# johndpope/MegaPortrait-hack

Hardware: AMD Instinct MI355X
Metric: Gbase fwd hot-slice frames/sec @512^2 (96ch 16x64x64 volume) (higher is better)
Workload: dtype f16x3 (fp32 in/out, operands split into 2 f16 halves, 3 f16 MFMAs per product, fp32 accumulate; 3x3x3 convs that fill the chip run in the F(2,3) Winograd domain along W)

## Files before the change

include/mphip.h:

```cpp
#ifndef MPHIP_H
#define MPHIP_H

#include <stddef.h>
#include <stdint.h>

#define MPHIP_RANGE_FLOATS 4100

#ifdef __cplusplus
extern "C" {
#endif

#define MPHIP_OK 0
#define MPHIP_EINVAL (-1)
#define MPHIP_ELAUNCH (-2)
#define MPHIP_EWORKSPACE (-3)

#define MPHIP_ABI_VERSION 25
int mphip_version(void);
int mphip_graph_memsets_to_kernels(void *graph, int *replaced);
int mphip_graph_memset_nodes_left(void *graph, int *left);

int mphip_build_flags(void);
const char *mphip_last_error(void);

int mphip_rt_theta(const float *rotation_deg, const float *translation, float *theta, int B, int invert,
                   void *stream);

int mphip_warp_field_compose(const float *theta, const float *em, const float *base_tbl, float *w,
                             float *rt_out, float *em_out, int B, int eD, int eH, int eW, int G,
                             void *stream);

size_t mphip_warp_workspace_bytes(int B, int D, int H, int W);
size_t mphip_warp_corner_image_bytes(int B, int C);
int mphip_warp_corner_image(const float *v, void *img, size_t img_bytes, int B, int C, int D, int H, int W, void *stream);
int mphip_warp_volume_coords_img(const float *v, const float *coords, float *out, float *out_range, int B, int C, int D, int H, int W,
                                 void *workspace, size_t workspace_bytes, const void *img, void *stream);
int mphip_warp_volume(const float *v, const float *field, const float *lin_d, const float *lin_h,
                      const float *lin_w, float *out, float *coords_out, int32_t *idx_out, float *out_range, int B,
                      int C, int D, int H, int W, int fD, int fH, int fW, void *workspace, size_t workspace_bytes,
                      void *stream);

int mphip_warp_volume_dsum(const float *v, const float *field, const float *lin_d, const float *lin_h,
                           const float *lin_w, float *out, int B, int C, int D, int H, int W, int fD,
                           int fH, int fW, void *workspace, size_t workspace_bytes, void *stream);
int mphip_warp_volume_dsum_shared(const float *v, const float *field, const float *lin_d, const float *lin_h,
                                  const float *lin_w, float *out, int B, int C, int D, int H, int W, int fD,
                                  int fH, int fW, void *workspace, size_t workspace_bytes, void *stream);

int mphip_conv3d_supported(int N, int Ci, int Co, int D, int H, int W, int k, int precision);
size_t mphip_packed_weight_bytes(int Co, int Ci, int k, int precision);
int mphip_pack_conv_weight(const float *w_oidhw, void *w_packed, int Co, int Ci, int k, int precision,
                           void *stream);
size_t mphip_conv3d_workspace_bytes(int N, int Ci, int Co, int D, int H, int W, int k, int precision);
int mphip_absmax_range(const float *x, size_t n, float *range, void *stream);
int mphip_conv3d_fwd(const float *x, const float *x_range, const void *w_packed, const float *bias, float *y, int N,
                     int Ci, int Co, int D, int H, int W, int k, int precision, void *workspace,
                     size_t workspace_bytes, void *stream);

size_t mphip_conv3d_gn_workspace_bytes(int N, int Ci, int Co, int D, int H, int W, int k, int precision,
                                       int gn_groups);
int mphip_conv3d_gn_fwd(const float *x, const float *x_range, const void *w_packed, const float *bias, float *y, float *gn_stats,
                        int N, int Ci, int Co, int D, int H, int W, int k, int precision, int gn_groups,
                        float gn_eps, void *workspace, size_t workspace_bytes, void *stream);

int mphip_groupnorm_affine_table(const float *stats, const float *gamma, const float *beta, const float *w2,
                                 const float *b2, float *table, float *out_range, int N, int C, int S, int G,
                                 void *stream);
int mphip_conv3d_gn_table_fwd(const float *x, const float *x_range, const void *w_packed, const float *bias, float *y, float *gn_stats,
                              const float *gamma, const float *beta, const float *w2, const float *b2, float *table, float *table_range,
                              int N, int Ci, int Co, int D, int H, int W, int k, int precision, int gn_groups, float gn_eps,
                              void *workspace, size_t workspace_bytes, void *stream);
int mphip_flowfield_conv_gn_supported(int Ci, int Co, int D, int H, int W, int Cr, int groups);
int mphip_flowfield_conv_gn(const float *x, const float *w, const float *b, const float *gamma, const float *beta, const float *w2,
                            const float *b2, const float *res_x, const float *res_w, const float *res_b, float *y, int N, int Ci, int Co,
                            int D, int H, int W, int Cr, int uD, int uH, int uW, int groups, float eps, int relu, void *stream);
size_t mphip_flowfield_compact_weight_bytes(int Ci, int Co, int D, int H, int W);
int mphip_flowfield_compact_weight(const float *w, void *w_compact, int Ci, int Co, void *stream);
int mphip_flowfield_conv_gn_compact(const float *x, const void *w_compact, const float *b, const float *gamma, const float *beta, const float *w2,
                                    const float *b2, const float *res_x, const float *res_w, const float *res_b, float *y, int N, int Ci, int Co,
                                    int D, int H, int W, int Cr, int uD, int uH, int uW, int groups, float eps, int relu, void *stream);
size_t mphip_flowfield_out_workspace_bytes(int N);
int mphip_flowfield_out(const float *x, const float *w, const float *b, const float *gamma, const float *beta, float *em, int N, float eps,
                        void *workspace, size_t workspace_bytes, void *stream);
void mphip_conv3d_time_next_launch(void *event_begin, void *event_end);
int mphip_conv3d_gnin_fwd(const float *x, const float *in_affine, const float *x_range, int in_relu, const void *w_packed,
                          const float *bias, float *y, int N, int Ci, int Co, int D, int H, int W, int k,
                          int precision, void *workspace, size_t workspace_bytes, void *stream);
int mphip_conv3d_gnin_gn_fwd(const float *x, const float *in_affine, const float *x_range, int in_relu, const void *w_packed,
                             const float *bias, float *y, float *gn_stats, int N, int Ci, int Co, int D, int H, int W,
                             int k, int precision, int gn_groups, float gn_eps, void *workspace,
                             size_t workspace_bytes, void *stream);

int mphip_conv3d_splits(int N, int Ci, int Co, int D, int H, int W, int k, int precision);
int mphip_conv3d_fwd_split(const float *x, const float *x_range, const void *w_packed, const float *bias, float *out,
                           int N, int Ci, int Co, int D, int H, int W, int k, int precision, void *workspace,
                           size_t workspace_bytes, void *stream);

size_t mphip_groupnorm_workspace_bytes(int N, int C, int S, int G);
int mphip_groupnorm_stats(const float *x, float *stats, int N, int C, int S, int G, float eps,
                          void *workspace, size_t workspace_bytes, void *stream);
int mphip_groupnorm_apply(const float *x, const float *stats, const float *gamma, const float *beta,
                          const float *w2, const float *b2, const float *residual, float *y, float *out_range, int N,
                          int C, int D, int H, int W, int G, int relu, int tanh_, int pool2, void *stream);

int mphip_groupnorm_stats_split(const float *x, int x_splits, const float *x_bias, float *stats, int N, int C,
                                int S, int G, float eps, void *stream);
int mphip_groupnorm_apply_split(const float *x, int x_splits, const float *x_bias, const float *stats,
                                const float *gamma, const float *beta, const float *w2, const float *b2,
                                const float *residual, int res_splits, const float *res_bias, float *y,
                                float *out_range, int N, int C, int D, int H, int W, int G, int relu, int tanh_,
                                int pool2, int uD, int uH, int uW, void *stream);

int mphip_groupnorm_small_fused(const float *x, int x_splits, const float *x_bias, const float *gamma,
                                const float *beta, const float *w2, const float *b2, const float *residual,
                                int res_splits, const float *res_bias, float *y, float *stats_out, int N, int C,
                                int D, int H, int W, int G, float eps, int relu, int tanh_, int uD, int uH, int uW,
                                void *stream);

int mphip_avgpool2(const float *x, float *y, int NC, int D, int H, int W, void *stream);
int mphip_upsample_trilinear2(const float *x, float *y, int NC, int D, int H, int W, void *stream);
int mphip_upsample_nearest(const float *x, float *y, int NC, int D, int H, int W, int sD, int sH, int sW,
                           void *stream);
int mphip_upsample_trilinear(const float *x, float *y, int NC, int D, int H, int W, int sD, int sH, int sW, void *stream);
int mphip_upsample_trilinear_bwd(const float *dout, float *dx, int NC, int D, int H, int W, int sD, int sH, int sW,
                                 void *stream);

int mphip_add_matmul(const float *a, const float *a2, const float *m, const float *bias, float *out, int B,
                     int K, int N, int trans, void *stream);

size_t mphip_grad_prep_workspace_bytes(int N, int C, int S);
int mphip_grad_prep(const float *dy, float *dbias, float *scale, int N, int C, int S, void *workspace,
                    size_t workspace_bytes, void *stream);
int mphip_pack_conv_weight_bwd_data(const float *w, void *wp, int Co, int Ci, int k, int precision, void *stream);
int mphip_pack_conv_weight_bwd_data_like(const float *w, void *wp, int Co, int Ci, int k, int precision,
                                         const void *fwd_pack, void *stream);
int mphip_conv3d_bwd_data(const float *dy, const void *wt_packed, float *dx, const float *dy_scale, int N, int Ci,
                          int Co, int D, int H, int W, int k, int precision, void *workspace, size_t workspace_bytes,
                          void *stream);
typedef struct mphip_pack_job {
    const float *w;
    void *wp;
    const void *like;
    int Co, Ci, k, precision, transposed;
} mphip_pack_job;
int mphip_pack_table_create(const mphip_pack_job *jobs, int n, void **table);
int mphip_pack_table_run(void *table, void *stream);
int mphip_pack_table_destroy(void *table);
int mphip_conv3d_bwd_weight_supported(int N, int Ci, int Co, int D, int H, int W, int k, int precision);
size_t mphip_conv3d_bwd_weight_workspace_bytes(int N, int Ci, int Co, int D, int H, int W, int k, int precision);
int mphip_conv3d_bwd_weight(const float *x, const float *x_range, const float *dy, const float *dy_scale, float *dw, int N,
                            int Ci, int Co, int D, int H, int W, int k, int precision, void *workspace,
                            size_t workspace_bytes, void *stream);
size_t mphip_groupnorm_bwd_workspace_bytes(int N, int C, int S);
int mphip_groupnorm_bwd_reduce(const float *x, const float *y, const float *dy, const float *stats,
// ... 178 lines not shown
```

megaportrait-hack_amd/_lib.py:

```python
from __future__ import annotations

import ctypes
import os
import subprocess

_HERE = os.path.dirname(os.path.abspath(__file__))
LIB_PATH = os.environ.get("MPHIP_LIB", os.path.join(_HERE, "libmphip.so"))
BUILD_SCRIPT = os.path.join(_HERE, "csrc", "build.sh")

_c_float_p = ctypes.c_void_p
_i = ctypes.c_int
_sz = ctypes.c_size_t
_p = ctypes.c_void_p

class PackJob(ctypes.Structure):
    _fields_ = [("w", ctypes.c_void_p), ("wp", ctypes.c_void_p), ("like", ctypes.c_void_p), ("Co", ctypes.c_int), ("Ci", ctypes.c_int),
                ("k", ctypes.c_int), ("precision", ctypes.c_int), ("transposed", ctypes.c_int)]


SIGNATURES = {
    "mphip_version": (_i, []),
    "mphip_last_error": (ctypes.c_char_p, []),
    "mphip_rt_theta": (_i, [_p, _p, _p, _i, _i, _p]),
    "mphip_warp_field_compose": (_i, [_p, _p, _p, _p, _p, _p, _i, _i, _i, _i, _i, _p]),
    "mphip_warp_workspace_bytes": (_sz, [_i, _i, _i, _i]),
    "mphip_warp_corner_image_bytes": (_sz, [_i, _i]),
    "mphip_warp_corner_image": (_i, [_p, _p, _sz] + [_i] * 5 + [_p]),
    "mphip_warp_volume_coords_img": (_i, [_p] * 4 + [_i] * 5 + [_p, _sz, _p, _p]),
    "mphip_warp_volume": (_i, [_p, _p, _p, _p, _p, _p, _p, _p, _p, _i, _i, _i, _i, _i, _i, _i, _i, _p, _sz, _p]),
    "mphip_warp_volume_dsum": (_i, [_p, _p, _p, _p, _p, _p, _i, _i, _i, _i, _i, _i, _i, _i, _p, _sz, _p]),
    "mphip_warp_volume_dsum_shared": (_i, [_p, _p, _p, _p, _p, _p, _i, _i, _i, _i, _i, _i, _i, _i, _p, _sz, _p]),
    "mphip_warp_volume_typed": (_i, [_p, _i, _p, _p, _p, _p, _p, _p, _p, _p] + [_i] * 8 + [_p, _sz, _p]),
    "mphip_warp_corner_image_typed": (_i, [_p, _i, _p, _sz] + [_i] * 5 + [_p]),
    "mphip_warp_volume_coords_img_typed": (_i, [_p, _i, _p, _p, _p] + [_i] * 5 + [_p, _sz, _p, _p]),
    "mphip_warp_volume_dsum_typed": (_i, [_p, _i, _p, _p, _p, _p, _p, _i] + [_i] * 8 + [_p, _sz, _p]),
    "mphip_warp_volume_dsum_coords_typed": (_i, [_p, _p, _p, _i] + [_i] * 5 + [_i, _p]),
    "mphip_cast_to_f32_range": (_i, [_p, _i, _sz, _p, _p, _p]),
    "mphip_cast_from_f32": (_i, [_p, _p, _i, _sz, _p]),
    "mphip_hot_slice_forward_typed": (_i, [_p, _p, _i] + [_p] * 7 + [_p, _i, _i, _p, _sz, _p]),
    "mphip_g3d_workspace_bytes_typed": (_sz, [_p, _i, _i, _i]),
    "mphip_g3d_forward_typed": (_i, [_p, _p, _i, _p, _p, _i, _i, _p, _sz, _p]),
    "mphip_conv3d_supported": (_i, [_i, _i, _i, _i, _i, _i, _i, _i]),
    "mphip_packed_weight_bytes": (_sz, [_i, _i, _i, _i]),
    "mphip_pack_conv_weight": (_i, [_p, _p, _i, _i, _i, _i, _p]),
    "mphip_conv3d_workspace_bytes": (_sz, [_i, _i, _i, _i, _i, _i, _i, _i]),
    "mphip_absmax_range": (_i, [_p, _sz, _p, _p]),
    "mphip_conv3d_fwd": (_i, [_p, _p, _p, _p, _p, _i, _i, _i, _i, _i, _i, _i, _i, _p, _sz, _p]),
    "mphip_conv3d_gn_workspace_bytes": (_sz, [_i, _i, _i, _i, _i, _i, _i, _i, _i]),
    "mphip_conv3d_gn_fwd": (_i, [_p, _p, _p, _p, _p, _p, _i, _i, _i, _i, _i, _i, _i, _i, _i, ctypes.c_float, _p, _sz, _p]),
    "mphip_conv3d_gn_table_fwd": (_i, [_p] * 12 + [_i] * 9 + [ctypes.c_float, _p, _sz, _p]),
    "mphip_conv3d_time_next_launch": (None, [_p, _p]),
    "mphip_groupnorm_affine_table": (_i, [_p, _p, _p, _p, _p, _p, _p, _i, _i, _i, _i, _p]),
    "mphip_conv3d_gnin_gn_fwd": (_i, [_p, _p, _p, _i, _p, _p, _p, _p] + [_i] * 9 + [ctypes.c_float, _p, _sz, _p]),
    "mphip_conv3d_gnin_fwd": (_i, [_p, _p, _p, _i, _p, _p, _p, _i, _i, _i, _i, _i, _i, _i, _i, _p, _sz, _p]),
    "mphip_conv3d_splits": (_i, [_i, _i, _i, _i, _i, _i, _i, _i]),
    "mphip_conv3d_fwd_split": (_i, [_p, _p, _p, _p, _p, _i, _i, _i, _i, _i, _i, _i, _i, _p, _sz, _p]),
    "mphip_groupnorm_stats_split": (_i, [_p, _i, _p, _p, _i, _i, _i, _i, ctypes.c_float, _p]),
    "mphip_groupnorm_apply_split": (_i, [_p, _i, _p, _p, _p, _p, _p, _p, _p, _i, _p, _p, _p] + [_i] * 12 + [_p]),
    "mphip_groupnorm_small_fused": (_i, [_p, _i, _p, _p, _p, _p, _p, _p, _i, _p, _p, _p] + [_i] * 6 + [ctypes.c_float] + [_i] * 5 + [_p]),
    "mphip_groupnorm_workspace_bytes": (_sz, [_i, _i, _i, _i]),
    "mphip_groupnorm_stats": (_i, [_p, _p, _i, _i, _i, _i, ctypes.c_float, _p, _sz, _p]),
    "mphip_groupnorm_apply": (_i, [_p, _p, _p, _p, _p, _p, _p, _p, _p, _i, _i, _i, _i, _i, _i, _i, _i, _i, _p]),
    "mphip_avgpool2": (_i, [_p, _p, _i, _i, _i, _i, _p]),
    "mphip_upsample_trilinear2": (_i, [_p, _p, _i, _i, _i, _i, _p]),
    "mphip_upsample_nearest": (_i, [_p, _p, _i, _i, _i, _i, _i, _i, _i, _p]),
    "mphip_upsample_trilinear": (_i, [_p, _p, _i, _i, _i, _i, _i, _i, _i, _p]),
    "mphip_upsample_trilinear_bwd": (_i, [_p, _p, _i, _i, _i, _i, _i, _i, _i, _p]),
    "mphip_add_matmul": (_i, [_p, _p, _p, _p, _p, _i, _i, _i, _i, _p]),
    "mphip_grad_prep_workspace_bytes": (_sz, [_i, _i, _i]),
    "mphip_grad_prep": (_i, [_p, _p, _p, _i, _i, _i, _p, _sz, _p]),
    "mphip_pack_conv_weight_bwd_data": (_i, [_p, _p, _i, _i, _i, _i, _p]),
    "mphip_pack_conv_weight_bwd_data_like": (_i, [_p, _p, _i, _i, _i, _i, _p, _p]),
    "mphip_conv3d_bwd_data": (_i, [_p, _p, _p, _p] + [_i] * 8 + [_p, _sz, _p]),
    "mphip_conv3d_bwd_weight_supported": (_i, [_i] * 8),
    "mphip_conv3d_bwd_weight_workspace_bytes": (_sz, [_i] * 8),
    "mphip_conv3d_bwd_weight": (_i, [_p, _p, _p, _p, _p] + [_i] * 8 + [_p, _sz, _p]),
    "mphip_groupnorm_bwd_workspace_bytes": (_sz, [_i, _i, _i]),
    "mphip_groupnorm_bwd_reduce": (_i, [_p] * 12 + [_i] * 5 + [_p, _sz, _p]),
    "mphip_groupnorm_bwd_apply": (_i, [_p] * 9 + [_i] * 5 + [_p]),
    "mphip_groupnorm_bwd": (_i, [_p] * 13 + [_i] * 5 + [_p, _sz, _p]),
    "mphip_upsample_nearest_bwd": (_i, [_p, _p] + [_i] * 7 + [_p]),
    "mphip_small_gemm": (_i, [_p] * 5 + [_i] * 3 + [ctypes.c_long] * 4 + [_p]),
    "mphip_warp_coords": (_i, [_p] * 5 + [_i] * 7 + [_p]),
    "mphip_warp_volume_bwd_workspace_bytes": (_sz, [_i] * 5),
    "mphip_warp_volume_bwd": (_i, [_p] * 8 + [_i] * 9 + [_p, _sz, _p]),
    "mphip_warp_field_compose_bwd_workspace_bytes": (_sz, [_i, _i]),
    "mphip_warp_field_compose_bwd": (_i, [_p] * 4 + [_i] * 5 + [_p, _sz, _p]),
    "mphip_rt_theta_bwd": (_i, [_p] * 5 + [_i, _i, _p]),
    "mphip_f16x3_saturation_count": (_i, [_p, _i]),
    "mphip_conv3d_set_half_products": (_i, [_i]),
    "mphip_avgpool2_bwd": (_i, [_p, _p, _i, _i, _i, _i, _p]),
    "mphip_upsample_trilinear2_bwd_workspace_bytes": (_sz, [_i] * 4),
    "mphip_upsample_trilinear2_bwd": (_i, [_p, _p, _i, _i, _i, _i, _p, _sz, _p]),
    "mphip_warp_field_coords": (_i, [_p] * 7 + [_i] * 6 + [_p]),
    "mphip_flowfield_conv_gn_supported": (_i, [_i] * 7),
    "mphip_flowfield_out_workspace_bytes": (_sz, [_i]),
    "mphip_flowfield_out": (_i, [_p] * 6 + [_i, ctypes.c_float, _p, _sz, _p]),
    "mphip_flowfield_conv_gn": (_i, [_p] * 11 + [_i] * 11 + [ctypes.c_float, _i, _p]),
    "mphip_flowfield_compact_weight_bytes": (_sz, [_i] * 5),
    "mphip_flowfield_compact_weight": (_i, [_p, _p, _i, _i, _p]),
    "mphip_flowfield_conv_gn_compact": (_i, [_p] * 11 + [_i] * 11 + [ctypes.c_float, _i, _p]),
    "mphip_warp_volume_coords": (_i, [_p] * 4 + [_i] * 5 + [_p, _sz, _p]),
    "mphip_warp_sample_box": (_i, [_p, _p, _i, _i, _i, _i, _p]),
    "mphip_conv3d_roi_granule": (_i, [_i] * 8 + [_p]),
    "mphip_conv3d_roi_workspace_bytes": (_sz, [_i] * 8),
    "mphip_conv3d_fwd_roi": (_i, [_p] * 6 + [_i] * 9 + [_p, _sz, _p]),
    "mphip_conv3d_bwd_data_roi": (_i, [_p] * 5 + [_i] * 8 + [_p, _sz, _p]),
    "mphip_conv3d_bwd_weight_roi": (_i, [_p] * 6 + [_i] * 8 + [_p, _sz, _p]),
    "mphip_upsample_trilinear2_roi": (_i, [_p, _p, _p] + [_i] * 9 + [_p]),
    "mphip_warp_volume_dsum_coords": (_i, [_p, _p, _p] + [_i] * 6 + [_p]),
    "mphip_hot_slice_plan_create": (_i, [_p, _p, _i, _i, _i, _i, _i, _i, _p]),
    "mphip_hot_slice_plan_set_tables": (_i, [_p, _p, _p, _p, _p]),
    "mphip_hot_slice_plan_refresh": (_i, [_p, _p, _p, _i]),
    "mphip_hot_slice_plan_profile": (_i, [_p, _i]),
    "mphip_hot_slice_plan_profile_read": (_i, [_p, _i, _p, _p]),
    "mphip_hot_slice_plan_set_precision": (_i, [_p, _i]),
    "mphip_hot_slice_workspace_bytes": (_sz, [_p, _i]),
    "mphip_hot_slice_forward": (_i, [_p] * 10 + [_i, _p, _sz, _p]),
    "mphip_g3d_workspace_bytes": (_sz, [_p, _i]),
    "mphip_g3d_forward": (_i, [_p, _p, _p, _p, _i, _p, _sz, _p]),
    "mphip_hot_slice_plan_destroy": (None, [_p]),
    "mphip_debug_mfma_sol": (_i, [_p, _i, _i, _i, _p]),
    "mphip_conv3d_kernel_variant": (_i, [_i] * 8),
    "mphip_debug_conv3d_plan": (_i, [_i] * 7 + [ctypes.POINTER(ctypes.c_int)]),
    "mphip_debug_conv3d_f32_plan": (_i, [_i] * 7 + [ctypes.POINTER(ctypes.c_int)]),
    "mphip_debug_conv3d_bwd_weight_f32_kernel": (_i, [_i] * 8 + [ctypes.POINTER(ctypes.c_int)]),
    "mphip_g2d_final_workspace_bytes": (_sz, [_i] * 6),
    "mphip_g2d_final_fwd": (_i, [_p, _i, _p, _p, _p, _p, _p, _i, _p] + [_i] * 6 + [ctypes.c_float, _p, _sz, _p]),
    "mphip_g2d_final_bwd": (_i, [_p] * 12 + [_i] * 6 + [_p, _sz, _p]),
    "mphip_conv2d_supported": (_i, [_i] * 5),
    "mphip_conv2d_packed_weight_bytes": (_sz, [_i, _i]),
    "mphip_pack_conv2d_weight": (_i, [_p, _p, _i, _i, _p]),
# ... 95 lines not shown
```

megaportrait-hack_amd/csrc/conv3d.hip:

```cpp
#include <stdlib.h>
#include <string.h>

#include <algorithm>
#include <vector>

#include "mphip_common.h"
#include "mphip_conv.h"

namespace mphip {

typedef float f32x16 __attribute__((ext_vector_type(16)));

__device__ __forceinline__ float buf_load(__amdgpu_buffer_rsrc_t rsrc, unsigned voff, unsigned soff) {
    return buf_load_f(rsrc, voff, soff);
}

__device__ __forceinline__ void pack_weight_body(const float *__restrict__ w, float *__restrict__ wp, int Co, int Ci, int CoP,
                                                 int CiP, int taps, int transposed, unsigned bid, unsigned nblk) {
    size_t n = (size_t)taps * CiP * CoP;
    for (size_t i = (size_t)bid * blockDim.x + threadIdx.x; i < n; i += (size_t)nblk * blockDim.x) {
        int co = (int)(i % CoP);
        int ci = (int)((i / CoP) % CiP);
        int tap = (int)(i / ((size_t)CoP * CiP));
        const size_t src = transposed ? ((size_t)ci * Co + co) * taps + (taps - 1 - tap) : ((size_t)co * Ci + ci) * taps + tap;
        wp[i] = (co < Co && ci < Ci) ? w[src] : 0.0f;
    }
}
__global__ void pack_weight_kernel(const float *__restrict__ w, float *__restrict__ wp, int Co, int Ci, int CoP,
                                   int CiP, int taps, int transposed) {
    pack_weight_body(w, wp, Co, Ci, CoP, CiP, taps, transposed, blockIdx.x, gridDim.x);
}
__global__ void __launch_bounds__(256) pack_many_f32_kernel(const PackJob *__restrict__ jobs, const int *__restrict__ sel,
                                                            const int *__restrict__ first, int n) {
    int lo = 0, hi = n - 1;
    while (lo < hi) {
        const int mid = (lo + hi + 1) >> 1;
        if (first[mid] <= (int)blockIdx.x) lo = mid; else hi = mid - 1;
    }
    const PackJob j = jobs[sel[lo]];
    pack_weight_body(j.w, (float *)j.wp, j.Co, j.Ci, (j.Co + 31) / 32 * 32, (j.Ci + 1) / 2 * 2, j.k * j.k * j.k, j.transposed,
                     blockIdx.x - first[lo], first[lo + 1] - first[lo]);
}

template <int KS, int MT, int NT, int WCO, bool SKIP>
__global__ void __launch_bounds__(256)
conv3d_gather_kernel(const float *__restrict__ x, const float *__restrict__ wp, const float *__restrict__ bias,
                     float *__restrict__ y, int N, int Ci, int CiP, int Co, int CoP, int D, int H, int W,
                     int ci_per_split, unsigned x_bytes) {
    MPHIP_LATENCY_KERNEL_PRIO();
    constexpr int TAPS = KS * KS * KS;
    constexpr int WVOX = 4 / WCO;
    const int lane = threadIdx.x & 63;
    const int wave = __builtin_amdgcn_readfirstlane(threadIdx.x >> 6);
    const int wave_co = wave % WCO, wave_vox = wave / WCO;
    const int j = lane & 31, kk = lane >> 5;
    const int HW = H * W, DHW = D * HW;
    const long M = (long)N * DHW;

    const int co0 = (blockIdx.y * WCO + wave_co) * MT * 32;
    const long v0 = ((long)blockIdx.x * WVOX + wave_vox) * NT * 32;
    if (co0 >= CoP || v0 >= M) return;

    const int ci_begin = blockIdx.z * ci_per_split;
    const int ci_end = min(CiP, ci_begin + ci_per_split);

    __amdgpu_buffer_rsrc_t rsrc = __builtin_amdgcn_make_buffer_rsrc((void *)x, 0, (int)x_bytes, 0x00020000);

    unsigned vbyte[NT];
    unsigned vmask[NT];
    unsigned anymask = 0;
#pragma unroll
    for (int t = 0; t < NT; ++t) {
        long vg = v0 + t * 32 + j;
        bool ok = vg < M;
        long vv = ok ? vg : 0;
        int n = (int)(vv / DHW);
        int r = (int)(vv - (long)n * DHW);
        int d = r / HW, h = (r / W) % H, w = r % W;
        vbyte[t] = (unsigned)(((long)n * Ci * DHW + (long)kk * DHW + r) * 4);
        unsigned m = 0;
        if (ok) {
#pragma unroll
            for (int tap = 0; tap < TAPS; ++tap) {
                int kd = KS == 3 ? tap / 9 - 1 : 0, kh = KS == 3 ? (tap / 3) % 3 - 1 : 0, kw = KS == 3 ? tap % 3 - 1 : 0;
                bool in = (unsigned)(d + kd) < (unsigned)D && (unsigned)(h + kh) < (unsigned)H &&
                          (unsigned)(w + kw) < (unsigned)W;
                m |= in ? (1u << tap) : 0u;
            }
        }
        vmask[t] = m;
// ... 693 lines not shown
    MPHIP_REQUIRE(roi_frames >= 0 && (roi_frames == 0 || N == 1), "conv3d_fwd_roi: roi_frames > 0 (several boxes on one volume) needs N == 1");
    int dims[3];
    const bool tiled = mphip_conv3d_roi_granule(N, Ci, Co, D, H, W, k, precision, dims) != 0;
    return conv3d_run(x, nullptr, 0, x_range, w_packed, bias, y, nullptr, 0, 0.0f, false, N, Ci, Co, D, H, W, k, precision, workspace,
                      workspace_bytes, stream, tiled ? roi : nullptr, tiled ? roi_frames : 0);
}

extern "C" int mphip_conv3d_kernel_variant(int N, int Ci, int Co, int D, int H, int W, int k, int precision) {
    F16x3Plan fp;
    if (!f16x3_plan_for(f16x3_switches(), fp, N, Ci, Co, D, H, W, k, precision, false)) return 0;
    return f16x3_is_wino(fp.kernel) ? 5 : 1;
}

extern "C" int mphip_debug_conv3d_plan(int N, int Ci, int Co, int D, int H, int W, int roi, int out[12]) {
    if (!out) return 0;
    for (int i = 0; i < 12; ++i) out[i] = 0;
    F16x3Plan fp;
    if (!f16x3_plan_for(f16x3_switches(), fp, N, Ci, Co, D, H, W, 3, 1, roi != 0)) return 0;
    const int v[12] = {(int)fp.kernel, fp.tile[0], fp.tile[1], fp.tile[2], fp.gn_rows, fp.tile_list, fp.max_gn_ci, fp.splits,
                       fp.chunks_per_split, (int)fp.grid.x, (int)fp.grid.y, (int)fp.grid.z};
    for (int i = 0; i < 12; ++i) out[i] = v[i];
    return 1;
}

extern "C" int mphip_debug_conv3d_f32_plan(int N, int Ci, int Co, int D, int H, int W, int k, int out[10]) {
    if (!out) return 0;
    for (int i = 0; i < 10; ++i) out[i] = 0;
    if (!conv_supported(f16x3_switches(), N, Ci, Co, D, H, W, k, 0)) return 0;
    const ConvPlan p = plan_conv(N, Ci, Co, D, H, W, k);
    const int v[10] = {p.tiled, p.tiled ? 3 : p.MT, p.tiled ? p.tiled / 2 : p.NT, p.tiled ? 1 : p.WCO, (!p.tiled && p.skip) ? 1 : 0,
                       p.splits, p.ci_per_split, (int)p.grid.x, (int)p.grid.y, (int)p.grid.z};
    for (int i = 0; i < 10; ++i) out[i] = v[i];
    return 1;
}

extern "C" int mphip_conv3d_splits(int N, int Ci, int Co, int D, int H, int W, int k, int precision) {
    const F16x3Switches sw = f16x3_switches();
    if (!conv_supported(sw, N, Ci, Co, D, H, W, k, precision)) return 0;
    F16x3Plan fp;
    if (f16x3_plan_for(sw, fp, N, Ci, Co, D, H, W, k, precision, false)) return fp.splits;
    return precision == 1 ? 1 : plan_conv(N, Ci, Co, D, H, W, k).splits;
}

extern "C" int mphip_conv3d_fwd_split(const float *x, const float *x_range, const void *w_packed, const float *bias, float *out,
                                      int N, int Ci, int Co, int D, int H, int W, int k, int precision, void *workspace,
                                      size_t workspace_bytes, void *stream) {
    return conv3d_run(x, nullptr, 0, x_range, w_packed, bias, out, nullptr, 0, 0.0f, true, N, Ci, Co, D, H, W, k, precision, workspace,
                      workspace_bytes, stream);
}

extern "C" size_t mphip_conv3d_gn_workspace_bytes(int N, int Ci, int Co, int D, int H, int W, int k, int precision,
                                                  int gn_groups) {
    if (gn_groups <= 0 || Co % gn_groups) return 0;
    const F16x3Switches sw = f16x3_switches();
    F16x3Plan fp;
    const F16x3Plan *fpp = f16x3_plan_for(sw, fp, N, Ci, Co, D, H, W, k, precision, false) ? &fp : nullptr;
    const size_t ws = conv_supported(sw, N, Ci, Co, D, H, W, k, precision) ? conv_ws_bytes(fpp, N, Ci, Co, D, H, W, k, precision) : 0;
    return ws + conv_gn_bytes(sw, fpp, N, Co, D * H * W, gn_groups);
}

extern "C" int mphip_conv3d_gn_fwd(const float *x, const float *x_range, const void *w_packed, const float *bias, float *y, float *gn_stats,
                                   int N, int Ci, int Co, int D, int H, int W, int k, int precision, int gn_groups,
                                   float gn_eps, void *workspace, size_t workspace_bytes, void *stream) {
    MPHIP_REQUIRE(gn_stats, "conv3d_gn_fwd: null stats pointer");
    MPHIP_REQUIRE(gn_groups > 0 && Co > 0 && Co % gn_groups == 0, "conv3d_gn_fwd: Co=%d not divisible into %d groups", Co,
                  gn_groups);
    return conv3d_run(x, nullptr, 0, x_range, w_packed, bias, y, gn_stats, gn_groups, gn_eps, false, N, Ci, Co, D, H, W, k, precision, workspace,
                      workspace_bytes, stream);
}

extern "C" int mphip_conv3d_gn_table_fwd(const float *x, const float *x_range, const void *w_packed, const float *bias, float *y, float *gn_stats,
                                         const float *gamma, const float *beta, const float *w2, const float *b2, float *table,
                                         float *table_range, int N, int Ci, int Co, int D, int H, int W, int k, int precision, int gn_groups,
                                         float gn_eps, void *workspace, size_t workspace_bytes, void *stream) {
    MPHIP_REQUIRE(gn_stats && gamma && beta && table && table_range, "conv3d_gn_table_fwd: null pointer");
    MPHIP_REQUIRE((w2 == nullptr) == (b2 == nullptr), "conv3d_gn_table_fwd: w2/b2 must both be set or both NULL");
    MPHIP_REQUIRE(gn_groups > 0 && Co > 0 && Co % gn_groups == 0, "conv3d_gn_table_fwd: Co=%d not divisible into %d groups", Co, gn_groups);
    GnTable t;
    t.gamma = gamma; t.beta = beta; t.w2 = w2; t.b2 = b2; t.table = table; t.range = table_range;
    return conv3d_run(x, nullptr, 0, x_range, w_packed, bias, y, gn_stats, gn_groups, gn_eps, false, N, Ci, Co, D, H, W, k, precision, workspace,
                      workspace_bytes, stream, nullptr, 0, 0, &t);
}

extern "C" int mphip_conv3d_gnin_fwd(const float *x, const float *in_affine, const float *x_range, int in_relu, const void *w_packed,
                                     const float *bias, float *y, int N, int Ci, int Co, int D, int H, int W, int k,
                                     int precision, void *workspace, size_t workspace_bytes, void *stream) {
    MPHIP_REQUIRE(in_affine && x_range, "conv3d_gnin_fwd: null affine table / range descriptor (mphip_groupnorm_affine_table makes both)");
    return conv3d_run(x, in_affine, in_relu, x_range, w_packed, bias, y, nullptr, 0, 0.0f, false, N, Ci, Co, D, H, W, k, precision,
                      workspace, workspace_bytes, stream);
}

extern "C" int mphip_conv3d_gnin_gn_fwd(const float *x, const float *in_affine, const float *x_range, int in_relu, const void *w_packed,
                                        const float *bias, float *y, float *gn_stats, int N, int Ci, int Co, int D, int H,
                                        int W, int k, int precision, int gn_groups, float gn_eps, void *workspace,
                                        size_t workspace_bytes, void *stream) {
    MPHIP_REQUIRE(in_affine && x_range && gn_stats, "conv3d_gnin_gn_fwd: null pointer");
    MPHIP_REQUIRE(gn_groups > 0 && Co > 0 && Co % gn_groups == 0, "conv3d_gnin_gn_fwd: Co=%d not divisible into %d groups", Co,
                  gn_groups);
    return conv3d_run(x, in_affine, in_relu, x_range, w_packed, bias, y, gn_stats, gn_groups, gn_eps, false, N, Ci, Co, D, H, W, k,
                      precision, workspace, workspace_bytes, stream);
}

extern "C" int mphip_conv3d_bwd_data_roi(const float *dy, const void *wt_packed, float *dx, const float *dy_scale, const int *roi, int N,
                                         int Ci, int Co, int D, int H, int W, int k, int precision, void *workspace,
                                         size_t workspace_bytes, void *stream) {
    MPHIP_REQUIRE(roi && dx, "conv3d_bwd_data_roi: null pointer");
    MPHIP_REQUIRE(precision == 0 || dy_scale, "conv3d_bwd_data_roi: the f16x3 kernel needs the gradient scale of mphip_grad_prep");
    F16x3Plan fp;
    const bool tiled = f16x3_plan_for(f16x3_switches(), fp, N, Ci, Co, D, H, W, k, precision, true) && fp.splits == 1;
    if (tiled) zero_fill(dx, (size_t)N * Co * D * H * W * sizeof(float), (hipStream_t)stream);
    return conv3d_run(dy, nullptr, 0, precision == 1 ? dy_scale : nullptr, wt_packed, nullptr, dx, nullptr, 0, 0.0f, false, N, Ci, Co, D, H, W, k,
                      precision, workspace, workspace_bytes, stream, tiled ? roi : nullptr, 0, 1);
}

extern "C" int mphip_conv3d_bwd_data(const float *dy, const void *wt_packed, float *dx, const float *dy_scale, int N, int Ci,
                                     int Co, int D, int H, int W, int k, int precision, void *workspace,
                                     size_t workspace_bytes, void *stream) {
    MPHIP_REQUIRE(precision == 0 || dy_scale, "conv3d_bwd_data: the f16x3 kernel needs the gradient scale of mphip_grad_prep");
    return conv3d_run(dy, nullptr, 0, precision == 1 ? dy_scale : nullptr, wt_packed, nullptr, dx, nullptr, 0, 0.0f, false, N, Ci,
                      Co, D, H, W, k, precision, workspace, workspace_bytes, stream);
}
```

megaportrait-hack_amd/csrc/conv3d_f16x3.hip:

```cpp
#include <stdlib.h>

#include <algorithm>


#include "mphip_ablate.h"
#include "mphip_common.h"
#include "mphip_conv.h"
#include "mphip_f16x3.h"

namespace mphip {

constexpr float X_SCALE = 16.0f;

__device__ unsigned long long g_f16x3_saturated;

#ifdef MPHIP_PROFILE_PHASES
__device__ unsigned long long g_f16x3_prof[8];
#define PROF_DECL unsigned long long pt_ = __builtin_readcyclecounter(), pa_[7] = {0, 0, 0, 0, 0, 0, 0}
#define PROF_ADD(slot) { const unsigned long long n_ = __builtin_readcyclecounter(); pa_[slot] += n_ - pt_; pt_ = n_; }
#define PROF_FLUSH if ((threadIdx.x & 63) == 0) { for (int q_ = 0; q_ < 7; ++q_) atomicAdd(&g_f16x3_prof[q_], pa_[q_]); atomicAdd(&g_f16x3_prof[7], 1ull); }
#else
#define PROF_DECL
#define PROF_ADD(slot)
#define PROF_FLUSH
#endif

#define F16X3_SAT_COUNT(a_, b_) sat_ += !(fabsf((a_) * x_scale) <= F16_CLAMP) + !(fabsf((b_) * x_scale) <= F16_CLAMP);

__device__ __forceinline__ void f16x3_absmax_body(const float *__restrict__ w, size_t n, unsigned *__restrict__ hdr, unsigned bid, unsigned nblk) {
    float m = 0.0f;
    const size_t n4 = ((uintptr_t)w & 15) == 0 ? n / 4 : 0;
    const float4 *w4 = reinterpret_cast<const float4 *>(w);
    for (size_t i = (size_t)bid * blockDim.x + threadIdx.x; i < n4; i += (size_t)nblk * blockDim.x) {
        const float4 q = w4[i];
        m = fmaxf(fmaxf(m, fmaxf(fabsf(q.x), fabsf(q.y))), fmaxf(fabsf(q.z), fabsf(q.w)));
    }
    for (size_t i = n4 * 4 + (size_t)bid * blockDim.x + threadIdx.x; i < n; i += (size_t)nblk * blockDim.x)
        m = fmaxf(m, fabsf(w[i]));
#pragma unroll
    for (int s = 32; s >= 1; s >>= 1) m = fmaxf(m, __shfl_xor(m, s, 64));
    __shared__ float red[4];
    if ((threadIdx.x & 63) == 0) red[threadIdx.x >> 6] = m;
    __syncthreads();
    if (threadIdx.x == 0) {
        const unsigned mine = __float_as_uint(fmaxf(fmaxf(red[0], red[1]), fmaxf(red[2], red[3])));
        if (mine > __hip_atomic_load(hdr + 2, __ATOMIC_RELAXED, __HIP_MEMORY_SCOPE_AGENT)) atomicMax(hdr + 2, mine);
    }
}
__global__ void __launch_bounds__(256) f16x3_absmax_kernel(const float *__restrict__ w, size_t n, unsigned *__restrict__ hdr) {
    f16x3_absmax_body(w, n, hdr, blockIdx.x, gridDim.x);
}

constexpr int PK_CO = 32;
constexpr int PK_LDS_FLOATS = PK_CO * (F16X3_KC * 27 + 1);
static_assert(PK_LDS_FLOATS >= F16X3_KC * (PK_CO * 27 + 1), "pack tile");
__device__ __forceinline__ void
f16x3_pack_body(const float *__restrict__ w, _Float16 *__restrict__ out, const unsigned *hdr_in, float *__restrict__ hdr_out, int Co,
                int Ci, int transposed, _Float16 *__restrict__ wino_out ,
                const int block , float *__restrict__ tile ) {
    const float scale = weight_scale(hdr_in[2]);
    const int nchunks = Ci / F16X3_KC, subs = F16X3_COT / PK_CO;
    int bid = block;
    const int sub = bid % subs; bid /= subs;
    const int chunk = bid % nchunks;
    const int cot = bid / nchunks;
    const int cog0 = cot * F16X3_COT + sub * PK_CO, ci0 = chunk * F16X3_KC;
    const int run = transposed ? PK_CO * 27 : F16X3_KC * 27, pitch = run + 1;
    constexpr int NQ = PK_CO * F16X3_KC * 27 / 4, NIT = (NQ + 255) / 256;
    float4 v[NIT];
#pragma unroll
    for (int it = 0; it < NIT; ++it) {
        const int i = it * 256 + threadIdx.x;
        const int r = i / (run / 4), q = i % (run / 4);
        const size_t src = transposed ? ((size_t)(ci0 + r) * Co + cog0) * 27 : ((size_t)(cog0 + r) * Ci + ci0) * 27;
        if (i < NQ) v[it] = *reinterpret_cast<const float4 *>(w + src + 4 * q);
    }
#pragma unroll
    for (int it = 0; it < NIT; ++it) {
        const int i = it * 256 + threadIdx.x;
        if (i < NQ) {
            float *d = tile + (i / (run / 4)) * pitch + 4 * (i % (run / 4));
            d[0] = v[it].x; d[1] = v[it].y; d[2] = v[it].z; d[3] = v[it].w;
        }
    }
    __syncthreads();
    for (int i = threadIdx.x; i < F16X3_NG * F16X3_TG * 2 * PK_CO; i += 256) {
        const int co = i % PK_CO;
        int r = i / PK_CO;
        const int kg = r % 2; r /= 2;
        const int tg = r % F16X3_TG;
        const int g = r / F16X3_TG;
// ... 486 lines not shown
    PROF_FLUSH
}

__global__ void __launch_bounds__(1024)
roi_tile_list_kernel(const int *__restrict__ roi, int roi_frames, int tiles_total, int D, int H, int W, int TD, int TH, int TW,
                     int dilate, int *__restrict__ list) {
    __shared__ int cnt;
    if (threadIdx.x == 0) cnt = 0;
    __syncthreads();
    const int tiles_w = W / TW, tiles_h = H / TH, tiles_d = D / TD;
    for (int t = threadIdx.x; t < tiles_total; t += 1024) {
        int bid = t;
        const int w0 = (bid % tiles_w) * TW; bid /= tiles_w;
        const int h0 = (bid % tiles_h) * TH; bid /= tiles_h;
        const int d0 = (bid % tiles_d) * TD;
        const int n = bid / tiles_d;
        const int first = roi_frames > 0 ? 0 : n, count = roi_frames > 0 ? roi_frames : 1;
        bool need = false;
        for (int f = first; f < first + count && !need; ++f) {
            const int *b = roi + f * 8;
            need = w0 < b[0] + b[3] + dilate && w0 + TW > b[0] - dilate && h0 < b[1] + b[4] + dilate && h0 + TH > b[1] - dilate &&
                   d0 < b[2] + b[5] + dilate && d0 + TD > b[2] - dilate;
        }
        if (need) list[1 + atomicAdd(&cnt, 1)] = t;
    }
    __syncthreads();
    if (threadIdx.x == 0) list[0] = cnt;
}

template <int TD, int TH, int TW, int NWAVES, int GS>
__global__ void __launch_bounds__(NWAVES * 64) __attribute__((amdgpu_waves_per_eu(2, 2)))
conv3d_k3_f16x3_kernel(const float *__restrict__ x, const _Float16 *__restrict__ wslabs, const float *__restrict__ whdr,
                       const float *__restrict__ bias, float *__restrict__ y, int N, int Ci, int Co, int D, int H, int W,
                       int chunks_per_split, unsigned x_bytes, const float *__restrict__ in_affine, int in_relu,
                       const float *__restrict__ x_scale_p, int tiles_total, int xcd_aware, const int *__restrict__ roi, int roi_frames,
                       float *__restrict__ gn_part) {
    conv3d_k3_f16x3_body<TD, TH, TW, NWAVES, GS>(x, wslabs, whdr, bias, y, N, Ci, Co, D, H, W, chunks_per_split, x_bytes, in_affine,
                                                 in_relu, x_scale_p, tiles_total, xcd_aware, roi, roi_frames, gn_part);
}

template <int TD, int TH, int TW, int NWAVES, int GS>
__global__ void __launch_bounds__(NWAVES * 64) __attribute__((amdgpu_waves_per_eu(2, 2)))
conv3d_k3_f16x3_third_kernel(const float *__restrict__ x, const _Float16 *__restrict__ wslabs, const float *__restrict__ whdr,
                             const float *__restrict__ bias, float *__restrict__ y, int N, int Ci, int Co, int D, int H, int W,
                             int chunks_per_split, unsigned x_bytes, const float *__restrict__ in_affine, int in_relu,
                             const float *__restrict__ x_scale_p, int tiles_total, int xcd_aware, const int *__restrict__ roi, int roi_frames,
                             float *__restrict__ gn_part) {
    conv3d_k3_f16x3_body<TD, TH, TW, NWAVES, GS, 1>(x, wslabs, whdr, bias, y, N, Ci, Co, D, H, W, chunks_per_split, x_bytes, in_affine,
                                                    in_relu, x_scale_p, tiles_total, xcd_aware, roi, roi_frames, gn_part);
}



__device__ __forceinline__ void f16x3_pack_k1_body(const float *__restrict__ w, _Float16 *__restrict__ out, const unsigned *hdr_in,
                                                   float *__restrict__ hdr_out, int Co, int Ci, int transposed, unsigned bid, unsigned nblk) {
    const float scale = weight_scale(hdr_in[2]);
    const int nchunks = Ci / F16X3_KC;
    const size_t n = (size_t)(Co / F16X3_COT) * nchunks * (K1_SLAB_HALFS / 2);
    for (size_t i = (size_t)bid * blockDim.x + threadIdx.x; i < n; i += (size_t)nblk * blockDim.x) {
        size_t r = i;
        const int e = (int)(r % 8); r /= 8;
        const int co = (int)(r % F16X3_COT); r /= F16X3_COT;
        const int kg = (int)(r % 2); r /= 2;
        const int chunk = (int)(r % nchunks);
        const int cot = (int)(r / nchunks);
        const int ci = chunk * F16X3_KC + kg * 8 + e, cog = cot * F16X3_COT + co;
        _Float16 hi, lo;
        split_f16(w[transposed ? (size_t)ci * Co + cog : (size_t)cog * Ci + ci] * scale, hi, lo);
        const size_t slab = (size_t)cot * nchunks + chunk;
        const size_t inner = ((size_t)kg * F16X3_COT + co) * 8 + e;
        out[slab * K1_SLAB_HALFS + inner] = hi;
        out[slab * K1_SLAB_HALFS + K1_SLAB_HALFS / 2 + inner] = lo;
    }
    if (bid == 0 && threadIdx.x == 0) {
        hdr_out[0] = 1.0f / scale;
        hdr_out[1] = scale;
    }
}
__global__ void __launch_bounds__(256) f16x3_pack_k1_kernel(const float *__restrict__ w, _Float16 *__restrict__ out, const unsigned *hdr_in,
                                                            float *__restrict__ hdr_out, int Co, int Ci, int transposed) {
    f16x3_pack_k1_body(w, out, hdr_in, hdr_out, Co, Ci, transposed, blockIdx.x, gridDim.x);
}

template <int KS, int NTT = 2>
__global__ void __launch_bounds__(KS == 1 ? 256 : 64 * KS) __attribute__((amdgpu_waves_per_eu(2)))
conv3d_k1_f16x3_kernel(const float *__restrict__ x, const _Float16 *__restrict__ wslabs, const float *__restrict__ whdr,
                       const float *__restrict__ bias, float *__restrict__ y, int N, int Ci, int Co, int DHW, unsigned x_bytes,
                       const float *__restrict__ x_range) {
    constexpr int MT = 3, NT = NTT;
    float x_scale = X_SCALE, x_unscale = 1.0f / X_SCALE;
    if (x_range) range_scale_block(x_range, x_scale, x_unscale);
    const int lane = threadIdx.x & 63, wave = threadIdx.x >> 6;
    const int j = lane & 31, kg = lane >> 5;
    const long v0 = (KS == 1 ? (long)blockIdx.x * 4 + wave : (long)blockIdx.x) * (NT * 32);
    if (v0 >= (long)N * DHW) return;
    const int n = (int)(v0 / DHW), r0 = (int)(v0 - (long)n * DHW);
    const int cot = blockIdx.y, nchunks = Ci / F16X3_KC;
    const int cps = (nchunks + KS - 1) / KS;
    const int c_begin = KS == 1 ? 0 : wave * cps, c_end = KS == 1 ? nchunks : min(nchunks, c_begin + cps);
    __amdgpu_buffer_rsrc_t rsrc = __builtin_amdgcn_make_buffer_rsrc((void *)x, 0, (int)x_bytes, 0x00020000);
    const unsigned vbase = (unsigned)((((long)n * Ci + kg * 8) * DHW + r0 + j) * 4);
    const unsigned cstride = (unsigned)DHW * 4u;
    const _Float16 *wl = wslabs + (size_t)cot * nchunks * K1_SLAB_HALFS + (kg * F16X3_COT + j) * 8;

    f32x16 acc[MT][NT];
#pragma unroll
    for (int m = 0; m < MT; ++m)
#pragma unroll
        for (int t = 0; t < NT; ++t)
#pragma unroll
            for (int q = 0; q < 16; ++q) acc[m][t][q] = 0.0f;

    unsigned sat_ = 0;
    float xv[2][NT][8];
    half8 ah[2][MT], al[2][MT];
#define K1_LOAD(set, c_)                                                                                              \
    {                                                                                                                 \
        const unsigned soff_ = (unsigned)((long)(c_) * F16X3_KC * DHW * 4);                                           \
        _Pragma("unroll") for (int t = 0; t < NT; ++t)                                                                \
            _Pragma("unroll") for (int e = 0; e < 8; ++e)                                                             \
                xv[set][t][e] = buf_load_f(rsrc, vbase + (unsigned)t * 128u + (unsigned)e * cstride, soff_);          \
        const _Float16 *ws_ = wl + (size_t)(c_) * K1_SLAB_HALFS;                                                      \
        _Pragma("unroll") for (int m = 0; m < MT; ++m) {                                                              \
            ah[set][m] = *reinterpret_cast<const half8 *>(ws_ + m * 32 * 8);                                          \
            al[set][m] = *reinterpret_cast<const half8 *>(ws_ + K1_SLAB_HALFS / 2 + m * 32 * 8);                      \
        }                                                                                                             \
    }
#define K1_MFMA(set)                                                                                                  \
    {                                                                                                                 \
        half8 bh[NT], bl[NT];                                                                                         \
        _Pragma("unroll") for (int t = 0; t < NT; ++t)                                                                \
            _Pragma("unroll") for (int e = 0; e < 8; ++e) {                                                           \
                _Float16 h, l;                                                                                        \
                const float sv = xv[set][t][e] * x_scale;                                                             \
                sat_ += !(fabsf(sv) <= F16_CLAMP);                                                                    \
                split_f16(sv, h, l);                                                                                  \
                bh[t][e] = h;                                                                                         \
                bl[t][e] = l;                                                                                         \
            }                                                                                                         \
        _Pragma("unroll") for (int m = 0; m < MT; ++m)                                                                \
            _Pragma("unroll") for (int t = 0; t < NT; ++t)                                                            \
                acc[m][t] = __builtin_amdgcn_mfma_f32_32x32x16_f16(al[set][m], bh[t], acc[m][t], 0, 0, 0);            \
        _Pragma("unroll") for (int m = 0; m < MT; ++m)                                                                \
            _Pragma("unroll") for (int t = 0; t < NT; ++t)                                                            \
                acc[m][t] = __builtin_amdgcn_mfma_f32_32x32x16_f16(ah[set][m], bl[t], acc[m][t], 0, 0, 0);            \
        _Pragma("unroll") for (int m = 0; m < MT; ++m)                                                                \
            _Pragma("unroll") for (int t = 0; t < NT; ++t)                                                            \
                acc[m][t] = __builtin_amdgcn_mfma_f32_32x32x16_f16(ah[set][m], bh[t], acc[m][t], 0, 0, 0);            \
    }
    if (c_begin < c_end) K1_LOAD(0, c_begin)
    for (int c = c_begin; c < c_end; c += 2) {
        if (c + 1 < c_end) K1_LOAD(1, c + 1)
        K1_MFMA(0)
        if (c + 1 < c_end) {
            if (c + 2 < c_end) K1_LOAD(0, c + 2)
            K1_MFMA(1)
        }
    }
#undef K1_LOAD
#undef K1_MFMA
    const float unscale = whdr[0] * x_unscale;
    const int co0 = cot * F16X3_COT;
    if (KS == 1) {
#pragma unroll
        for (int m = 0; m < MT; ++m) {
#pragma unroll
            for (int reg = 0; reg < 16; ++reg) {
                const int co = co0 + m * 32 + (reg & 3) + 8 * (reg >> 2) + 4 * kg;
                const float bv = bias ? bias[co] : 0.0f;
                float *dv = y + ((size_t)n * Co + co) * DHW + r0 + j;
#pragma unroll
                for (int t = 0; t < NT; ++t) dv[t * 32] = acc[m][t][reg] * unscale + bv;
            }
        }
    } else {
        __shared__ float red[KS > 1 ? KS : 1][NT * 16 * 64];
#pragma unroll
        for (int m = 0; m < MT; ++m) {
#pragma unroll
            for (int t = 0; t < NT; ++t)
#pragma unroll
                for (int reg = 0; reg < 16; ++reg) red[wave][(t * 16 + reg) * 64 + lane] = acc[m][t][reg];
            __syncthreads();
            for (int q = wave; q < NT * 16; q += KS) {
                const int t = q >> 4, reg = q & 15;
                float sum = red[0][q * 64 + lane];
#pragma unroll
                for (int k = 1; k < KS; ++k) sum += red[k][q * 64 + lane];
                const int co = co0 + m * 32 + (reg & 3) + 8 * (reg >> 2) + 4 * kg;
                const float bv = bias ? bias[co] : 0.0f;
                y[((size_t)n * Co + co) * DHW + r0 + j + t * 32] = sum * unscale + bv;
            }
            __syncthreads();
        }
    }
    if (__builtin_amdgcn_ballot_w64(sat_ != 0) != 0) {
        unsigned tot = sat_;
#pragma unroll
        for (int sft = 32; sft >= 1; sft >>= 1) tot += __shfl_xor(tot, sft, 64);
        if (lane == 0) atomicAdd(&g_f16x3_saturated, (unsigned long long)tot);
    }
}

static int f16x3_k1_ksplit(const F16x3Switches &sw, int N, int Ci, int Co, int DHW) {
    if (sw.k1_ks == 1 || sw.k1_ks == 4 || sw.k1_ks == 8) return sw.k1_ks;
    const long wave_tiles = (long)N * DHW / 64 * (Co / F16X3_COT);
    const int nchunks = Ci / F16X3_KC;
    if (wave_tiles >= 1024 || nchunks < 8) return 1;
    return (wave_tiles <= 512 && nchunks >= 16) ? 8 : 4;
}

int f16x3_pack(const float *w, void *out, int Co, int Ci, int k, int transposed, const void *header_from, hipStream_t s) {
    const unsigned *hdr = (const unsigned *)out;
    if (header_from) {
        hdr = (const unsigned *)header_from;
    } else {
        zero_fill(out, 16, s);
        const size_t n = (size_t)Co * Ci * (k == 3 ? 27 : 1);
        hipLaunchKernelGGL(f16x3_absmax_kernel, dim3((unsigned)std::min<size_t>(2048, (n + 4095) / 4096)), dim3(256), 0, s, w, n,
                           (unsigned *)out);
    }
    if (k == 1)
        hipLaunchKernelGGL(f16x3_pack_k1_kernel, dim3(256), dim3(256), 0, s, w, (_Float16 *)((char *)out + 16), hdr, (float *)out, Co,
                           Ci, transposed);
    else {
        hipLaunchKernelGGL(f16x3_pack_kernel, dim3((unsigned)((Co / PK_CO) * (Ci / F16X3_KC))), dim3(256), 0, s, w,
                           (_Float16 *)((char *)out + 16), hdr, (float *)out, Co, Ci, transposed,
                           f16x3_wino_packed_bytes(Co, Ci) ? (_Float16 *)((char *)out + f16x3_direct_bytes(Co, Ci)) : (_Float16 *)nullptr);
    }
    return check_launch("pack_conv_weight(f16x3)");
}

__device__ __forceinline__ int pack_find(const int *__restrict__ first, int n, int bid) {
    int lo = 0, hi = n - 1;
    while (lo < hi) {
        const int mid = (lo + hi + 1) >> 1;
        if (first[mid] <= bid) lo = mid; else hi = mid - 1;
    }
    return lo;
}
__device__ __forceinline__ const unsigned *pack_hdr_in(const PackJob &j) { return (const unsigned *)(j.like ? j.like : j.wp); }
__global__ void __launch_bounds__(256) pack_many_zero_hdr_kernel(const PackJob *__restrict__ jobs, const int *__restrict__ sel, int n) {
    const int i = blockIdx.x * 256 + threadIdx.x;
    if (i < n * 4) reinterpret_cast<unsigned *>(jobs[sel[i >> 2]].wp)[i & 3] = 0u;
}
__global__ void __launch_bounds__(256) pack_many_absmax_kernel(const PackJob *__restrict__ jobs, const int *__restrict__ sel,
                                                               const int *__restrict__ first, int n) {
    const int q = pack_find(first, n, (int)blockIdx.x);
    const PackJob j = jobs[sel[q]];
    f16x3_absmax_body(j.w, (size_t)j.Co * j.Ci * (j.k == 3 ? 27 : 1), (unsigned *)j.wp, blockIdx.x - first[q], first[q + 1] - first[q]);
}
__global__ void __launch_bounds__(256) pack_many_k3_kernel(const PackJob *__restrict__ jobs, const int *__restrict__ sel,
                                                           const int *__restrict__ first, int n) {
    __shared__ __attribute__((aligned(16))) float tile[PK_LDS_FLOATS];
    const int q = pack_find(first, n, (int)blockIdx.x);
    const PackJob j = jobs[sel[q]];
    char *out = (char *)j.wp;
    f16x3_pack_body(j.w, (_Float16 *)(out + 16), pack_hdr_in(j), (float *)out, j.Co, j.Ci, j.transposed,
                    j.wino_off ? (_Float16 *)(out + j.wino_off) : (_Float16 *)nullptr,
                    (int)blockIdx.x - first[q], tile);
}
__global__ void __launch_bounds__(256) pack_many_k1_kernel(const PackJob *__restrict__ jobs, const int *__restrict__ sel,
                                                           const int *__restrict__ first, int n) {
    const int q = pack_find(first, n, (int)blockIdx.x);
    const PackJob j = jobs[sel[q]];
    char *out = (char *)j.wp;
    f16x3_pack_k1_body(j.w, (_Float16 *)(out + 16), pack_hdr_in(j), (float *)out, j.Co, j.Ci, j.transposed, blockIdx.x - first[q],
                       first[q + 1] - first[q]);
}

size_t f16x3_pack_wino_offset(int Co, int Ci) { return f16x3_wino_packed_bytes(Co, Ci) ? f16x3_direct_bytes(Co, Ci) : 0; }

int f16x3_pack_blocks(const PackJob &j, int kind) {
    const size_t n = (size_t)j.Co * j.Ci * (j.k == 3 ? 27 : 1);
    if (kind == 0) return (int)std::min<size_t>(2048, (n + 4095) / 4096);
    if (kind == 1) return (j.Co / PK_CO) * (j.Ci / F16X3_KC);
    return (int)std::min<size_t>(256, (n + 255) / 256);
}

int f16x3_pack_many(const PackJob *jobs, PackSel absmax, PackSel k3, PackSel k1, hipStream_t s) {
    if (absmax.n) {
        hipLaunchKernelGGL(pack_many_zero_hdr_kernel, dim3((unsigned)((absmax.n * 4 + 255) / 256)), dim3(256), 0, s, jobs, absmax.job, absmax.n);
        hipLaunchKernelGGL(pack_many_absmax_kernel, dim3((unsigned)absmax.blocks), dim3(256), 0, s, jobs, absmax.job, absmax.first, absmax.n);
    }
    if (k3.n) hipLaunchKernelGGL(pack_many_k3_kernel, dim3((unsigned)k3.blocks), dim3(256), 0, s, jobs, k3.job, k3.first, k3.n);
    if (k1.n) hipLaunchKernelGGL(pack_many_k1_kernel, dim3((unsigned)k1.blocks), dim3(256), 0, s, jobs, k1.job, k1.first, k1.n);
    return check_launch("pack_conv_weights(f16x3)");
}

int f16x3_launch_k1(const F16x3Switches &sw, const float *x, const void *wpacked, const float *bias, float *dst, int N, int Ci, int Co,
                    int DHW, const float *x_range, hipStream_t s) {
    const float *hdr = (const float *)wpacked;
    const _Float16 *slabs = (const _Float16 *)((const char *)wpacked + 16);
    const unsigned xb = (unsigned)((size_t)N * Ci * DHW * 4);
    const long waves = (long)N * DHW / 64;
    const int ks = f16x3_k1_ksplit(sw, N, Ci, Co, DHW);
    const bool nt1 = ks == 1 && (sw.k1_nt >= 0 ? sw.k1_nt == 1 : waves * (Co / F16X3_COT) <= 1024);
    if (ks == 8)
        hipLaunchKernelGGL(conv3d_k1_f16x3_kernel<8>, dim3((unsigned)waves, Co / F16X3_COT), dim3(512), 0, s, x, slabs, hdr, bias, dst, N, Ci,
                           Co, DHW, xb, x_range);
    else if (ks == 4)
        hipLaunchKernelGGL(conv3d_k1_f16x3_kernel<4>, dim3((unsigned)waves, Co / F16X3_COT), dim3(256), 0, s, x, slabs, hdr, bias, dst, N, Ci,
                           Co, DHW, xb, x_range);
    else if (nt1)
        hipLaunchKernelGGL((conv3d_k1_f16x3_kernel<1, 1>), dim3((unsigned)((2 * waves + 3) / 4), Co / F16X3_COT), dim3(256), 0, s, x, slabs, hdr,
                           bias, dst, N, Ci, Co, DHW, xb, x_range);
    else
        hipLaunchKernelGGL(conv3d_k1_f16x3_kernel<1>, dim3((unsigned)((waves + 3) / 4), Co / F16X3_COT), dim3(256), 0, s, x, slabs, hdr, bias,
                           dst, N, Ci, Co, DHW, xb, x_range);
    return check_launch("conv3d_fwd(f16x3, k=1)");
}

int f16x3_launch(const F16x3Switches &sw, const F16x3Plan &p, const float *x, const void *wpacked, const float *bias, float *dst, int N, int Ci,
                 int Co, int D, int H, int W, const float *in_affine, int in_relu, const float *x_scale, hipStream_t s, const int *roi,
                 int roi_frames, int *tile_list, int roi_dilate, float *gn_part, hipEvent_t t0, hipEvent_t t1) {
    const bool wino = f16x3_is_wino(p.kernel);
    if (in_affine && Ci > p.max_gn_ci) {
        set_error("conv3d_fwd(f16x3%s): fused input GroupNorm supports Ci <= %d (got %d)", wino ? ", F(2,3)" : "", p.max_gn_ci, Ci);
        return MPHIP_EINVAL;
    }
    if ((roi && !p.tile_list) || (gn_part && !p.gn_rows)) {
        set_error("conv3d_fwd(f16x3, F(2,3), D = 2): no demand-driven tile list / GroupNorm partials in the two-frame mode");
        return MPHIP_EINVAL;
    }
    const float *hdr = (const float *)wpacked;
    const _Float16 *slabs = (const _Float16 *)((const char *)wpacked + (wino ? f16x3_direct_bytes(Co, Ci) : 16));
    const unsigned xb = (unsigned)((size_t)N * Ci * D * H * W * 4);
    if (roi) {
        hipLaunchKernelGGL(roi_tile_list_kernel, dim3(1), dim3(1024), 0, s, roi, roi_frames, (int)p.grid.x, D, H, W, p.tile[0], p.tile[1], p.tile[2],
                           roi_dilate, tile_list);
        roi = tile_list;
    }
    const int tiles_total = (int)p.grid.x;
    const bool thirds = roi && p.kernel == F16X3_DIRECT_4 && !gn_part && !sw.thirds_off;
    const long others = (long)p.grid.y * (thirds ? 3 : 1) * p.grid.z;
    long gx = (sw.conv_cus * p.wgs_per_cu + others - 1) / others;
    if (gx < 1) gx = 1;
    if (gx > tiles_total || (sw.no_persist && !wino)) gx = tiles_total;
    const dim3 grid((unsigned)gx, p.grid.y * (thirds ? 3 : 1), p.grid.z);
    const int xcd_on = sw.xcd_on, cps = p.chunks_per_split;
    const F16x3ConvArgs a = {x, slabs, hdr, bias, dst, N, Ci, Co, D, H, W, cps, xb, in_affine, in_relu, x_scale, tiles_total, xcd_on, roi, gn_part};
    auto direct = [&](auto kern, int block) {
        launch_timed(kern, grid, dim3(block), s, t0, t1, a.x, a.slabs, a.hdr, a.bias, a.dst, N, Ci, Co, D, H, W, cps, xb, a.in_affine, in_relu,
                     a.x_range, tiles_total, xcd_on, a.tile_list, roi_frames, gn_part);
    };
    switch (p.kernel) {
        case F16X3_DIRECT_4:
            if (thirds) direct(conv3d_k3_f16x3_third_kernel<4, 8, 8, 8, 3>, 512);
            else direct(conv3d_k3_f16x3_kernel<4, 8, 8, 8, 3>, 512);
            return check_launch("conv3d_fwd(f16x3)");
        case F16X3_DIRECT_2:
            direct(conv3d_k3_f16x3_kernel<2, 8, 8, 4, 1>, 256);
            return check_launch("conv3d_fwd(f16x3)");
        case F16X3_WINO_LOCKSTEP:
            f16x3_wino_launch(grid, s, t0, t1, a);
            return check_launch("conv3d_fwd(f16x3, F(2,3))");
        case F16X3_WINO_ROLE_SPLIT:
            f16x3_wino_pp_launch(grid, s, t0, t1, a, p.one_product);
            return check_launch("conv3d_fwd(f16x3, F(2,3), role-split)");
        case F16X3_WINO_BIG_TILE:
            f16x3_wino_bt_launch(grid, s, t0, t1, a, false);
            return check_launch("conv3d_fwd(f16x3, F(2,3), big tile)");
        case F16X3_WINO_TWO_FRAME:
            f16x3_wino_bt_launch(grid, s, t0, t1, a, true);
            return check_launch("conv3d_fwd(f16x3, F(2,3), big tile, two frames)");
    }
    set_error("conv3d_fwd(f16x3): plan names no kernel");
    return MPHIP_EINVAL;
}

}

#ifdef MPHIP_PROFILE_PHASES
extern "C" int mphip_debug_f16x3_profile(unsigned long long *out8, int reset) {
    if (hipMemcpyFromSymbol(out8, HIP_SYMBOL(mphip::g_f16x3_prof), 64) != hipSuccess) return -1;
    if (reset) {
        unsigned long long z[8] = {0, 0, 0, 0, 0, 0, 0, 0};
        if (hipMemcpyToSymbol(HIP_SYMBOL(mphip::g_f16x3_prof), z, 64) != hipSuccess) return -1;
    }
    return 0;
}
#endif

extern "C" int mphip_f16x3_saturation_count(unsigned long long *count, int reset) {
    MPHIP_REQUIRE(count, "f16x3_saturation_count: null pointer");
    if (mphip::f16x3_counter_read(&mphip::g_f16x3_saturated, count, reset) != 0) {
        mphip::set_error("f16x3_saturation_count: reading the counter failed");
        return MPHIP_ELAUNCH;
    }
    for (auto other : {mphip::f16x3_wino_saturation, mphip::f16x3_wino_pp_saturation, mphip::f16x3_wino_bt_saturation,
                       mphip::conv2d_f16x3_saturation, mphip::conv2d_gn_f16x3_saturation, mphip::conv2d_lp_saturation,
                       mphip::conv2d_s2_saturation, mphip::conv2d_up2_saturation, mphip::conv2d_grp_saturation,
                       mphip::conv2d_split_saturation}) {
// ... 10 lines not shown
```

megaportrait-hack_amd/csrc/conv3d_f16x3_plan.hip:

```cpp
#include <stdlib.h>

#include "mphip_conv.h"

namespace mphip {

F16x3Switches f16x3_switches() {
    const auto zero = [](const char *name) { const char *e = getenv(name); return e && e[0] == '0'; };
    const auto num = [](const char *name, long unset) { const char *e = getenv(name); return e ? atol(e) : unset; };
    static const F16x3Switches fixed = [&] {
        F16x3Switches f{};
        f.old_splits = getenv("MPHIP_F16X3_OLD_SPLITS") != nullptr;
        f.xcd_on = !zero("MPHIP_F16X3_XCD");
        f.wino_nopack = zero("MPHIP_WINOGRAD_PACK");
        f.thirds_off = zero("MPHIP_ROI_THIRDS");
        f.conv_cus = num("MPHIP_CONV_CUS", 256);
        f.gn_epilogue_off = zero("MPHIP_GN_EPILOGUE");
        f.k1_nt = (int)num("MPHIP_F16X3_K1_NT", -1);
        return f;
    }();
    F16x3Switches sw = fixed;
    sw.direct_only = getenv("MPHIP_F16X3_TILE") != nullptr;
    sw.force_splits = (int)num("MPHIP_F16X3_SPLITS", 0);
    sw.no_persist = getenv("MPHIP_F16X3_NO_PERSIST") != nullptr;
    sw.wino_off = zero("MPHIP_WINOGRAD");
    sw.d2_off = zero("MPHIP_WINOGRAD_D2");
    sw.min_tiles_set = getenv("MPHIP_WINOGRAD_MIN_TILES") != nullptr;
    sw.min_tiles = num("MPHIP_WINOGRAD_MIN_TILES", 192);
    const char *pp = getenv("MPHIP_WINO_PP");
    sw.wino_pp = !pp ? 1 : pp[0] == '0' ? 0 : pp[0] == '2' ? 2 : 1;
    sw.k1_ks = (int)num("MPHIP_F16X3_K1_KS", 0);
    sw.k1_min_voxels = num("MPHIP_F16X3_K1_MIN", 1024);
    return sw;
}

bool f16x3_supported(const F16x3Switches &sw, int N, int Ci, int Co, int D, int H, int W, int k) {
    if (k == 1)
        return Ci % F16X3_KC == 0 && Co % F16X3_COT == 0 && ((long)D * H * W) % 64 == 0 && (long)N * D * H * W >= sw.k1_min_voxels &&
               (size_t)N * Ci * D * H * W * 4 < 0x80000000ull;
    return k == 3 && Ci % F16X3_KC == 0 && Co % F16X3_COT == 0 && H % 8 == 0 && W % 8 == 0 && D % 2 == 0 &&
           (size_t)N * Ci * D * H * W * 4 < 0x80000000ull;
}

size_t f16x3_packed_bytes_k1(int Co, int Ci) {
    return 16 + (size_t)(Co / F16X3_COT) * (Ci / F16X3_KC) * K1_SLAB_HALFS * sizeof(_Float16);
}

size_t f16x3_direct_bytes(int Co, int Ci) {
    return 16 + (size_t)(Co / F16X3_COT) * (Ci / F16X3_KC) * F16X3_NG * SLAB_HALFS * sizeof(_Float16);
}

static size_t wino_packed_bytes(const F16x3Switches &sw, int Co, int Ci) {
    if (sw.wino_nopack || Ci % WN_KC || Co % WN_COT || Ci > 2 * WN_AFF_CI) return 0;
    return (size_t)(Co / WN_COT) * (Ci / WN_KC) * WN_NG * WN_SLAB_HALFS * sizeof(_Float16);
}
size_t f16x3_wino_packed_bytes(int Co, int Ci) { return wino_packed_bytes(f16x3_switches(), Co, Ci); }

size_t f16x3_packed_bytes(int Co, int Ci) {
    return f16x3_direct_bytes(Co, Ci) + f16x3_wino_packed_bytes(Co, Ci);
}

static int split_k(long base, int nchunks, long slots) {
    int sp = 1;
    if (base < slots)
        for (int dv = 2; dv <= nchunks; ++dv)
            if (nchunks % dv == 0 && base * dv <= slots) sp = dv;
    return sp;
}

static long wino_tiles(int N, int D, int H, int W) {
    return D == 2 ? (long)((N + 1) / 2) * (H / WN_TH) * (W / WN_TW) : (long)N * (D / WN_TD) * (H / WN_TH) * (W / WN_TW);
}

static int wino_splits(const F16x3Switches &sw, int N, int Ci, int Co, int D, int H, int W, bool roi) {
    if (sw.direct_only || sw.wino_off || wino_packed_bytes(sw, Co, Ci) == 0 || H % WN_TH || W % WN_TW) return 0;
    if (D == 2) {
        if (roi || sw.d2_off || (N < 4 && !sw.min_tiles_set)) return 0;
    } else if (D % WN_TD || Ci > WN_AFF_CI) {
        return 0;
    }
    const long base = wino_tiles(N, D, H, W) * (Co / WN_COT);
    const int sp = split_k(base, Ci / WN_KC, 256);
    return base * sp >= sw.min_tiles ? sp : 0;
}

F16x3Plan f16x3_plan(const F16x3Switches &sw, int N, int Ci, int Co, int D, int H, int W, bool roi, bool half_products) {
    F16x3Plan p{};
    const int cot = Co / F16X3_COT, nchunks = Ci / F16X3_KC;
    long tiles;
    p.tile[1] = p.tile[2] = 8;
    p.tile_list = true;
    p.max_gn_ci = F16X3_AFF_CI;
    p.wgs_per_cu = 1;
    if (const int wsp = wino_splits(sw, N, Ci, Co, D, H, W, roi)) {
        p.kernel = D == 2 ? F16X3_WINO_TWO_FRAME : (sw.wino_pp == 2 && !half_products) ? F16X3_WINO_BIG_TILE
                 : sw.wino_pp != 0 ? F16X3_WINO_ROLE_SPLIT : F16X3_WINO_LOCKSTEP;
        p.one_product = half_products && p.kernel == F16X3_WINO_ROLE_SPLIT;
        p.tile[0] = WN_TD;
        if (p.kernel == F16X3_WINO_TWO_FRAME) {
            p.gn_rows = 0;
            p.tile_list = false;
        } else {
            p.gn_rows = 2;
            p.max_gn_ci = WN_AFF_CI;
        }
        tiles = wino_tiles(N, D, H, W);
        p.splits = wsp;
    } else {
        const int td = D % 4 == 0 ? 4 : 2;
        p.kernel = td == 4 ? F16X3_DIRECT_4 : F16X3_DIRECT_2;
        p.tile[0] = td;
        p.gn_rows = td == 4 ? 8 : 4;
        p.wgs_per_cu = td == 4 ? 1 : 2;
        tiles = (long)N * (D / td) * (H / 8) * (W / 8);
        const long base = tiles * cot;
// ... 17 lines not shown
```

megaportrait-hack_amd/csrc/mphip_conv.h:

```cpp
#pragma once
#include <hip/hip_ext.h>

#include "mphip_common.h"

namespace mphip {

constexpr unsigned OOB = 0x80000000u;

__device__ __forceinline__ float buf_load_f(__amdgpu_buffer_rsrc_t rsrc, unsigned voff, unsigned soff) {
    return __builtin_bit_cast(float, __builtin_amdgcn_raw_buffer_load_b32(rsrc, (int)voff, (int)soff, 0));
}

typedef float mphip_f32x4 __attribute__((ext_vector_type(4)));
__device__ __forceinline__ mphip_f32x4 buf_load_f4(__amdgpu_buffer_rsrc_t rsrc, unsigned voff, unsigned soff) {
    typedef unsigned u32x4_ __attribute__((ext_vector_type(4)));
    return __builtin_bit_cast(mphip_f32x4, (u32x4_)__builtin_amdgcn_raw_buffer_load_b128(rsrc, (int)voff, (int)soff, 0));
}

constexpr int F16X3_KC = 16;
constexpr int F16X3_TG = 3;
constexpr int F16X3_NG = 27 / F16X3_TG;
constexpr int F16X3_COT = 96;
constexpr int SLAB_HALFS = 2 * F16X3_TG * 2 * F16X3_COT * 8;
constexpr int K1_SLAB_HALFS = 2 * 2 * F16X3_COT * 8;
constexpr int F16X3_AFF_CI = 768;
constexpr int WN_KC = 16;
constexpr int WN_COT = 96;
constexpr int WN_NG = 9;
constexpr int WN_SLAB_HALFS = 2 * 4 * 2 * WN_COT * 8;
constexpr int WN_TD = 4, WN_TH = 8, WN_TW = 8;
constexpr int WN_AFF_CI = 384;

struct F16x3Switches {
    bool direct_only;
    int force_splits;
    bool no_persist;
    bool wino_off;
    bool d2_off;
    bool min_tiles_set;
    long min_tiles;
    int wino_pp;
    int k1_ks;
    long k1_min_voxels;
    bool old_splits;
    bool xcd_on;
    bool wino_nopack;
    bool thirds_off;
    long conv_cus;
    bool gn_epilogue_off;
    int k1_nt;
};
F16x3Switches f16x3_switches();

enum F16x3Kernel {
    F16X3_DIRECT_2,
    F16X3_DIRECT_4,
    F16X3_WINO_LOCKSTEP,
    F16X3_WINO_ROLE_SPLIT,
    F16X3_WINO_BIG_TILE,
    F16X3_WINO_TWO_FRAME,
};
inline bool f16x3_is_wino(F16x3Kernel k) { return k >= F16X3_WINO_LOCKSTEP; }

struct F16x3Plan {
    F16x3Kernel kernel;
    int tile[3];
    int gn_rows;
    bool tile_list;
    bool one_product;
    int max_gn_ci;
    int wgs_per_cu;
    int splits, chunks_per_split;
    dim3 grid;
};
F16x3Plan f16x3_plan(const F16x3Switches &sw, int N, int Ci, int Co, int D, int H, int W, bool roi, bool half_products);

bool f16x3_supported(const F16x3Switches &sw, int N, int Ci, int Co, int D, int H, int W, int k);
size_t f16x3_direct_bytes(int Co, int Ci);
size_t f16x3_packed_bytes(int Co, int Ci);
size_t f16x3_packed_bytes_k1(int Co, int Ci);
int f16x3_launch_k1(const F16x3Switches &sw, const float *x, const void *wpacked, const float *bias, float *dst, int N, int Ci, int Co,
                    int DHW, const float *x_range, hipStream_t s);
int f16x3_pack(const float *w_oidhw, void *out, int Co, int Ci, int k, int transposed, const void *header_from, hipStream_t s);
struct PackJob {
    const float *w;
    void *wp;
    const void *like;
    size_t wino_off;
    int Co, Ci, k, precision, transposed, reserved;
};
struct PackSel {
    const int *job;
    const int *first;
    int n, blocks;
};
int f16x3_pack_blocks(const PackJob &j, int kind );
size_t f16x3_pack_wino_offset(int Co, int Ci);
int f16x3_pack_many(const PackJob *jobs, PackSel absmax, PackSel k3, PackSel k1, hipStream_t s);
int f16x3_launch(const F16x3Switches &sw, const F16x3Plan &p, const float *x, const void *wpacked, const float *bias, float *dst, int N, int Ci,
                 int Co, int D, int H, int W, const float *in_affine, int in_relu, const float *x_range, hipStream_t s,
                 const int *roi = nullptr, int roi_frames = 0, int *tile_list = nullptr , int roi_dilate = 0,
                 float *gn_part = nullptr ,
                 hipEvent_t t0 = nullptr, hipEvent_t t1 = nullptr );

template <class K, class... A>
void launch_timed(K kern, dim3 grid, dim3 block, hipStream_t s, hipEvent_t t0, hipEvent_t t1, A... args) {
    if (t0 && t1) hipExtLaunchKernelGGL(kern, grid, block, 0, s, t0, t1, 0, args...);
    else hipLaunchKernelGGL(kern, grid, block, 0, s, args...);
}

struct F16x3ConvArgs {
    const float *x;
    const _Float16 *slabs;
    const float *hdr, *bias;
    float *dst;
    int N, Ci, Co, D, H, W, cps;
    unsigned xb;
    const float *in_affine;
    int in_relu;
    const float *x_range;
    int tiles, xcd_on;
    const int *tile_list;
    float *gn_part;
};
template <class K>
void f16x3_wino_launch_kernel(K kern, dim3 grid, dim3 block, hipStream_t s, hipEvent_t t0, hipEvent_t t1, const F16x3ConvArgs &a) {
    launch_timed(kern, grid, block, s, t0, t1, a.x, a.slabs, a.hdr, a.bias, a.dst, a.N, a.Ci, a.Co, a.D, a.H, a.W, a.cps, a.xb, a.in_affine,
                 a.in_relu, a.x_range, a.tiles, a.xcd_on, a.tile_list, a.gn_part);
}

size_t f16x3_wino_packed_bytes(int Co, int Ci);
void f16x3_wino_launch(dim3 grid, hipStream_t s, hipEvent_t t0, hipEvent_t t1, const F16x3ConvArgs &a);
int f16x3_wino_saturation(unsigned long long *count, int reset);
void f16x3_wino_pp_launch(dim3 grid, hipStream_t s, hipEvent_t t0, hipEvent_t t1, const F16x3ConvArgs &a, bool half_products);
int f16x3_wino_pp_saturation(unsigned long long *count, int reset);
void f16x3_wino_bt_launch(dim3 grid, hipStream_t s, hipEvent_t t0, hipEvent_t t1, const F16x3ConvArgs &a, bool two_frame);
int f16x3_wino_bt_saturation(unsigned long long *count, int reset);
int conv2d_f16x3_saturation(unsigned long long *count, int reset);
int conv2d_gn_f16x3_saturation(unsigned long long *count, int reset);
int conv2d_lp_saturation(unsigned long long *count, int reset);
int conv2d_s2_saturation(unsigned long long *count, int reset);
int conv2d_up2_saturation(unsigned long long *count, int reset);
int conv2d_grp_saturation(unsigned long long *count, int reset);
int conv2d_split_saturation(unsigned long long *count, int reset);

struct C2Call {
    const char *who;
    int stride;
    int up2;
    int groups;
    int splits;
    bool cat;
    const void *x1, *x2;
    const float *aff1, *aff2, *x1_range, *x2_range;
    int relu1, relu2, C1, C2;
    int x_dtype, residual_dtype, y_dtype;
    int products;
    const void *w_packed;
    const float *bias;
    const void *residual;
    void *y;
    float *out_range;
    int N, Co, H, W, relu;
    void *workspace;
    size_t workspace_bytes;
// ... 46 lines not shown
```

megaportrait-hack_amd/csrc/norm.hip:

```cpp
#include <stdlib.h>

#include "mphip_common.h"
#include "mphip_conv.h"
#include "mphip_resample.h"

namespace mphip {

constexpr int GN_CHUNK = 16384;

__device__ __forceinline__ double wave_sum(double v) {
#pragma unroll
    for (int s = 32; s >= 1; s >>= 1) v += __shfl_xor(v, s, 64);
    return v;
}


__device__ __forceinline__ void gn_span_moments(const float *__restrict__ p, size_t begin, size_t end, bool vec, float k, float &s, float &ss) {
    if (vec) {
#pragma unroll 8
        for (size_t i = begin + (size_t)threadIdx.x * 4; i < end; i += 1024) {
            float4 v = *reinterpret_cast<const float4 *>(p + i);
            v.x -= k; v.y -= k; v.z -= k; v.w -= k;
            s += (v.x + v.y) + (v.z + v.w);
            ss += (v.x * v.x + v.y * v.y) + (v.z * v.z + v.w * v.w);
        }
    } else {
        for (size_t i = begin + threadIdx.x; i < end; i += 256) {
            float v = p[i] - k;
            s += v;
            ss += v * v;
        }
    }
}

__device__ __forceinline__ void gn_pivot_moments(double a, double b, double cnt, double k, double &mean, double &var) {
    const double d = a / cnt;
    mean = k + d;
    var = b / cnt - d * d;
    if (var < 0.0) var = 0.0;
}

__global__ void __launch_bounds__(256)
gn_partial_kernel(const float *__restrict__ x, double *__restrict__ partial, size_t cnt, int chunks) {
    const int grp = blockIdx.y, chunk = blockIdx.x;
    const float *p = x + (size_t)grp * cnt;
    const size_t begin = (size_t)chunk * GN_CHUNK;
    const size_t end = begin + GN_CHUNK < cnt ? begin + GN_CHUNK : cnt;
    const float k = p[0];
    float s = 0.0f, ss = 0.0f;
    gn_span_moments(p, begin, end, (cnt & 3) == 0 && (((size_t)p) & 15) == 0, k, s, ss);
    double ds = wave_sum((double)s), dss = wave_sum((double)ss);
    __shared__ double red[8];
    const int wave = threadIdx.x >> 6, lane = threadIdx.x & 63;
    if (lane == 0) {
        red[wave * 2] = ds;
        red[wave * 2 + 1] = dss;
    }
    __syncthreads();
    if (threadIdx.x == 0) {
        double a = (red[0] + red[2]) + (red[4] + red[6]);
        double b = (red[1] + red[3]) + (red[5] + red[7]);
        partial[((size_t)grp * chunks + chunk) * 2] = a;
        partial[((size_t)grp * chunks + chunk) * 2 + 1] = b;
    }
}

constexpr int GN_DIRECT_CHUNKS = 4;

__device__ __forceinline__ unsigned gn_table_entry(const GnTable &t, int n, int c, float mean, float rstd) {
    float scale = rstd * t.gamma[c];
    float shift = t.beta[c] - mean * scale;
    float amp = t.gamma[c], off = t.beta[c];
    if (t.w2) {
        scale = scale * t.w2[c];
        shift = shift * t.w2[c] + t.b2[c];
        amp = amp * t.w2[c];
        off = off * t.w2[c] + t.b2[c];
    }
    const int i = n * t.C + c;
    t.table[i * 2] = scale;
    t.table[i * 2 + 1] = shift;
    return range_bits((t.sqrt_ng * fabsf(amp) + fabsf(off)) * 1.0001f);
}

__device__ __forceinline__ void gn_block_span_stats(const float *__restrict__ p, size_t cnt, double &mean, double &var) {
    const bool vec = (cnt & 3) == 0 && (((size_t)p) & 15) == 0;
// ... 27 lines not shown
    const int grp = blockIdx.x;
    double mean, var;
    gn_block_span_stats(x + (size_t)grp * cnt, cnt, mean, var);
    __shared__ float mr_[2];
    if (threadIdx.x == 0) {
        stats[grp * 2] = mr_[0] = (float)mean;
        stats[grp * 2 + 1] = mr_[1] = (float)(1.0 / sqrt(var + (double)eps));
    }
    if (tbl.table) {
        __syncthreads();
        const int groups = tbl.C / tbl.cpg, n = grp / groups, g = grp % groups;
        unsigned mbits = 0;
        if ((int)threadIdx.x < tbl.cpg) mbits = gn_table_entry(tbl, n, g * tbl.cpg + threadIdx.x, mr_[0], mr_[1]);
        if (tbl.range) range_note_block(mbits, tbl.range, blockIdx.x, gridDim.x);
    }
}

__global__ void __launch_bounds__(1024)
gn_stats_split_kernel(const float *__restrict__ x, int splits, size_t slab, const float *__restrict__ bias,
                      float *__restrict__ stats, int C, int cpg, int S, float eps) {
    const int grp = blockIdx.x;
    const size_t cnt = (size_t)cpg * S, base = (size_t)grp * cnt;
    const int c0 = (int)((base / S) % (size_t)C);
    float k = sum_slabs(x, splits, slab, base);
    if (bias) k += bias[c0];
    double ds = 0.0, dss = 0.0;
    {
        float s = 0.0f, ss = 0.0f;
#pragma unroll 4
        for (size_t e = threadIdx.x; e < cnt; e += blockDim.x) {
            const size_t o = base + e;
            float v = sum_slabs(x, splits, slab, o);
            if (bias) v += bias[c0 + (int)(e / S)];
            v -= k;
            s += v;
            ss += v * v;
        }
        ds = (double)s;
        dss = (double)ss;
    }
    ds = wave_sum(ds);
    dss = wave_sum(dss);
    __shared__ double red[32];
    const int wave = threadIdx.x >> 6, lane = threadIdx.x & 63, nwaves = blockDim.x >> 6;
    if (lane == 0) {
        red[wave * 2] = ds;
        red[wave * 2 + 1] = dss;
    }
    __syncthreads();
    if (threadIdx.x == 0) {
        double a = 0.0, b = 0.0;
        for (int w = 0; w < nwaves; w += 4) {
            a += (red[w * 2] + red[w * 2 + 2]) + (red[w * 2 + 4] + red[w * 2 + 6]);
            b += (red[w * 2 + 1] + red[w * 2 + 3]) + (red[w * 2 + 5] + red[w * 2 + 7]);
        }
        double mean, var;
        gn_pivot_moments(a, b, (double)cnt, (double)k, mean, var);
        stats[grp * 2] = (float)mean;
        stats[grp * 2 + 1] = (float)(1.0 / sqrt(var + (double)eps));
    }
}

__global__ void gn_finalize_kernel(const float *__restrict__ x, const double *__restrict__ partial, float *__restrict__ stats, int ngroups,
                                   int chunks, double cnt, float eps, GnTable tbl) {
    int g = blockIdx.x * blockDim.x + threadIdx.x;
    unsigned mbits = 0;
    if (g < ngroups) {
        double s = 0.0, ss = 0.0;
        for (int c = 0; c < chunks; ++c) {
            s += partial[((size_t)g * chunks + c) * 2];
            ss += partial[((size_t)g * chunks + c) * 2 + 1];
        }
        double mean, var;
        gn_pivot_moments(s, ss, cnt, (double)x[(size_t)g * (size_t)cnt], mean, var);
        const float mf = (float)mean, rf = (float)(1.0 / sqrt(var + (double)eps));
        stats[g * 2] = mf;
        stats[g * 2 + 1] = rf;
        if (tbl.table) {
            const int groups = tbl.C / tbl.cpg, n = g / groups, gg = g % groups;
            for (int k = 0; k < tbl.cpg; ++k) mbits = max(mbits, gn_table_entry(tbl, n, gg * tbl.cpg + k, mf, rf));
        }
    }
    if (tbl.table && tbl.range) range_note_block(mbits, tbl.range, blockIdx.x, gridDim.x);
}

struct GnParams {
    const float *x, *stats, *gamma, *beta, *w2, *b2, *residual;
    float *y;
    int C, cpg;
    int relu, tanh_;
    float *range;
};

__device__ __forceinline__ float gn_value(const GnParams &p, float xv, float mean, float rstd, float g, float b,
                                          float w2, float b2, bool has2, float res, bool has_res) {
    float v = (xv - mean) * rstd * g + b;
    if (has2) v = v * w2 + b2;
    if (has_res) v += res;
    if (p.relu) v = fmaxf(v, 0.0f);
    if (p.tanh_) v = tanhf(v);
    return v;
}

template <int VW>
__global__ void __launch_bounds__(256) gn_apply_kernel(GnParams p, int S, size_t total_vec) {
    unsigned mbits = 0;
    for (size_t t = (size_t)blockIdx.x * blockDim.x + threadIdx.x; t < total_vec; t += (size_t)gridDim.x * blockDim.x) {
        const int SV = S / VW;
        size_t plane = t / SV;
        int c = (int)(plane % p.C);
        int n = (int)(plane / p.C);
        int grp = n * (p.C / p.cpg) + c / p.cpg;
        float mean = p.stats[grp * 2], rstd = p.stats[grp * 2 + 1];
        float g = p.gamma[c], b = p.beta[c];
        bool has2 = p.w2 != nullptr, has_res = p.residual != nullptr;
        float w2 = has2 ? p.w2[c] : 1.0f, b2 = has2 ? p.b2[c] : 0.0f;
        size_t o = t * VW;
        if (VW == 4) {
            float4 xv = *reinterpret_cast<const float4 *>(p.x + o);
            float4 rv = has_res ? *reinterpret_cast<const float4 *>(p.residual + o) : make_float4(0, 0, 0, 0);
            float4 out;
            out.x = gn_value(p, xv.x, mean, rstd, g, b, w2, b2, has2, rv.x, has_res);
            out.y = gn_value(p, xv.y, mean, rstd, g, b, w2, b2, has2, rv.y, has_res);
            out.z = gn_value(p, xv.z, mean, rstd, g, b, w2, b2, has2, rv.z, has_res);
            out.w = gn_value(p, xv.w, mean, rstd, g, b, w2, b2, has2, rv.w, has_res);
            *reinterpret_cast<float4 *>(p.y + o) = out;
            mbits = max(max(mbits, range_bits(out.x)), max(max(range_bits(out.y), range_bits(out.z)), range_bits(out.w)));
        } else {
            const float v = gn_value(p, p.x[o], mean, rstd, g, b, w2, b2, has2, has_res ? p.residual[o] : 0.0f, has_res);
            p.y[o] = v;
            mbits = max(mbits, range_bits(v));
        }
    }
    if (p.range) range_note_block(mbits, p.range, blockIdx.x, gridDim.x);
}

template <int PW>
__global__ void __launch_bounds__(256) gn_apply_pool_kernel(GnParams p, int D, int H, int W, size_t total) {
    unsigned mbits = 0;
    for (size_t t = (size_t)blockIdx.x * blockDim.x + threadIdx.x; t < total; t += (size_t)gridDim.x * blockDim.x) {
    const int oD = D / 2, oH = H / 2, oW = W / 2, oWp = oW / PW;
    int ow = (int)(t % oWp) * PW;
    size_t r = t / oWp;
    int oh = (int)(r % oH);
    r /= oH;
    int od = (int)(r % oD);
    size_t plane = r / oD;
    int c = (int)(plane % p.C);
    int n = (int)(plane / p.C);
    int grp = n * (p.C / p.cpg) + c / p.cpg;
    float mean = p.stats[grp * 2], rstd = p.stats[grp * 2 + 1];
    float g = p.gamma[c], b = p.beta[c];
    bool has2 = p.w2 != nullptr, has_res = p.residual != nullptr;
    float w2 = has2 ? p.w2[c] : 1.0f, b2 = has2 ? p.b2[c] : 0.0f;
    float s[PW];
#pragma unroll
    for (int q = 0; q < PW; ++q) s[q] = 0.0f;
#pragma unroll
    for (int a = 0; a < 2; ++a)
#pragma unroll
        for (int bb = 0; bb < 2; ++bb) {
            size_t o = ((plane * D + 2 * od + a) * H + 2 * oh + bb) * W + 2 * ow;
            float xv[2 * PW], rv[2 * PW];
            if (PW == 2) {
                const float4 x4 = *reinterpret_cast<const float4 *>(p.x + o);
                xv[0] = x4.x; xv[1] = x4.y; xv[2 * PW - 2] = x4.z; xv[2 * PW - 1] = x4.w;
                const float4 r4 = has_res ? *reinterpret_cast<const float4 *>(p.residual + o) : make_float4(0, 0, 0, 0);
                rv[0] = r4.x; rv[1] = r4.y; rv[2 * PW - 2] = r4.z; rv[2 * PW - 1] = r4.w;
            } else {
                xv[0] = p.x[o]; xv[1] = p.x[o + 1];
                rv[0] = has_res ? p.residual[o] : 0.0f; rv[1] = has_res ? p.residual[o + 1] : 0.0f;
            }
#pragma unroll
            for (int q = 0; q < PW; ++q) {
                s[q] += gn_value(p, xv[2 * q], mean, rstd, g, b, w2, b2, has2, rv[2 * q], has_res);
                s[q] += gn_value(p, xv[2 * q + 1], mean, rstd, g, b, w2, b2, has2, rv[2 * q + 1], has_res);
            }
        }
    const size_t oo = ((plane * oD + od) * oH + oh) * oW + ow;
    if (PW == 2) *reinterpret_cast<float2 *>(p.y + oo) = make_float2(s[0] / 8.0f, s[PW - 1] / 8.0f);
    else p.y[oo] = s[0] / 8.0f;
#pragma unroll
    for (int q = 0; q < PW; ++q) mbits = max(mbits, range_bits(s[q] / 8.0f));
    }
// ... 833 lines not shown
```

megaportrait-hack_amd/csrc/plan.hip:

```cpp
#include <stdlib.h>
#include <string.h>

#include <string>
#include <unordered_map>
#include <vector>

#include "linspace_tables.h"
#include "mphip_common.h"

using namespace mphip;

namespace {

constexpr float GN_EPS = 1e-5f;
constexpr size_t SPLIT_CHAIN_MAX_ELEMS = 1u << 18;
constexpr int SPLIT_CHAIN_MAX_SPLITS = 16;
constexpr size_t SPLIT_CHAIN_MAX_SLAB_ELEMS = 1u << 20;
constexpr size_t STATS_SPLIT_MAX_SPAN = 65536;
constexpr size_t GN_FUSED_MAX_SPAN = 12288;
constexpr size_t ALIGN = 256;

struct Arena {
    struct Block { size_t off, size; bool free; };
    std::vector<Block> blocks;
// ... 157 lines not shown
}

int precision_for(const Ctx &c, int n, int ci, int co, int d, int h, int w, int k) {
    if (c.p->precision == 0) return 0;
    return mphip_conv3d_supported(n, ci, co, d, h, w, k, 1) ? 1 : 0;
}

const void *packed(Ctx &c, ConvW &cw, int prec) {
    if (c.dry) return nullptr;
    if (!cw.pk[prec]) {
        const size_t bytes = mphip_packed_weight_bytes(cw.co, cw.ci, cw.k, prec);
        void *q = nullptr;
        if (bytes == 0 || hipMalloc(&q, bytes) != hipSuccess) {
            set_error("hot_slice: cannot allocate %zu bytes of packed weights (Co=%d Ci=%d k=%d precision %d)", bytes, cw.co, cw.ci, cw.k, prec);
            c.rc = MPHIP_ELAUNCH;
            return nullptr;
        }
        c.p->owned.push_back(q);
        cw.pk[prec] = q;
        cw.fresh[prec] = false;
    }
    if (!cw.fresh[prec] && !c.dry && c.rc == MPHIP_OK) {
        RUN(c, mphip_pack_conv_weight(cw.w, cw.pk[prec], cw.co, cw.ci, cw.k, prec, c.s));
        if (c.rc == MPHIP_OK) cw.fresh[prec] = true;
    }
    return cw.pk[prec];
}

void prof_arm(Ctx &c, const ConvW &cw, int d, int h, int w, int kind) {
    Plan *p = c.p;
    if (c.dry || c.rc != MPHIP_OK  || !p->profile || cw.ci != 96 || cw.co != 96 || cw.k != 3 || d != p->D || h != p->H || w != p->W) return;
    if (p->prof_used[kind] + 2 > p->prof_ev[kind].size())
        for (int i = 0; i < 2; ++i) {
            hipEvent_t e;
            if (hipEventCreate(&e) != hipSuccess) return;
            p->prof_ev[kind].push_back(e);
        }
    mphip_conv3d_time_next_launch(p->prof_ev[kind][p->prof_used[kind]], p->prof_ev[kind][p->prof_used[kind] + 1]);
    p->prof_used[kind] += 2;
}

const float *range_for(Ctx &c, T5 &x) {
    if (!x.has_range) {
        x.range = take(c, MPHIP_RANGE_FLOATS * sizeof(float));
        x.has_range = true;
        RUN(c, mphip_absmax_range(x.data.p, x.numel(), x.range.p, c.s));
    }
    return x.range.p;
}

bool gn_in_conv_ok(const Ctx &c, int n, int d, int h, int w, const ConvW &pc2);

ConvOut conv3d(Ctx &c, T5 &x, ConvW &cw, int gn_groups, const Norm *nm = nullptr, const ConvW *next = nullptr) {
    const int n = x.n, d = x.d, h = x.h, w = x.w;
    const int prec = precision_for(c, n, cw.ci, cw.co, d, h, w, cw.k);
    const void *wp = packed(c, cw, prec);
    const float *xr = prec == 1 ? range_for(c, x) : nullptr;
    const size_t ws_bytes = gn_groups ? mphip_conv3d_gn_workspace_bytes(n, cw.ci, cw.co, d, h, w, cw.k, prec, gn_groups)
                                      : mphip_conv3d_workspace_bytes(n, cw.ci, cw.co, d, h, w, cw.k, prec);
    Buf ws;
    if (ws_bytes) ws = take(c, ws_bytes);
    ConvOut o;
    o.t = new_t5(c, n, cw.co, d, h, w, false);
    prof_arm(c, cw, d, h, w, 0);
    if (gn_groups) {
        o.stats = take(c, (size_t)n * gn_groups * 2 * sizeof(float));
        o.stats_groups = gn_groups;
        if (nm && next && gn_in_conv_ok(c, n, d, h, w, *next)) {
            o.table = take(c, (size_t)n * cw.co * 2 * sizeof(float));
            o.table_range = take(c, MPHIP_RANGE_FLOATS * sizeof(float));
            RUN(c, mphip_conv3d_gn_table_fwd(x.data.p, xr, wp, cw.b, o.t.data.p, o.stats.p, nm->gw, nm->gb, nm->w2, nm->b2, o.table.p, o.table_range.p, n,
                                             cw.ci, cw.co, d, h, w, cw.k, prec, gn_groups, GN_EPS, ws.p, ws_bytes, c.s));
        } else {
            RUN(c, mphip_conv3d_gn_fwd(x.data.p, xr, wp, cw.b, o.t.data.p, o.stats.p, n, cw.ci, cw.co, d, h, w, cw.k, prec, gn_groups, GN_EPS,
                                       ws.p, ws_bytes, c.s));
        }
    } else {
        RUN(c, mphip_conv3d_fwd(x.data.p, xr, wp, cw.b, o.t.data.p, n, cw.ci, cw.co, d, h, w, cw.k, prec, ws.p, ws_bytes, c.s));
    }
    give(c, ws);
    return o;
}

ConvOut conv3d_split(Ctx &c, T5 &x, ConvW &cw, int gn_groups, const Norm *nm = nullptr, const ConvW *next = nullptr) {
    const int n = x.n, d = x.d, h = x.h, w = x.w;
    const int prec = precision_for(c, n, cw.ci, cw.co, d, h, w, cw.k);
    const int splits = mphip_conv3d_splits(n, cw.ci, cw.co, d, h, w, cw.k, prec);
    const size_t elems = (size_t)n * cw.co * d * h * w;
    if (splits > 1 && (elems > SPLIT_CHAIN_MAX_ELEMS || (splits >= SPLIT_CHAIN_MAX_SPLITS && (size_t)splits * elems > SPLIT_CHAIN_MAX_SLAB_ELEMS)))
        return conv3d(c, x, cw, gn_groups, nm, next);
    if (gn_groups && splits == 1 && prec == 1) return conv3d(c, x, cw, gn_groups, nm, next);
    const void *wp = packed(c, cw, prec);
    const float *xr = prec == 1 ? range_for(c, x) : nullptr;
    ConvOut o;
    o.t.n = n; o.t.c = cw.co; o.t.d = d; o.t.h = h; o.t.w = w;
    o.t.data = take(c, (size_t)splits * elems * sizeof(float));
    o.splits = splits;
    o.bias = splits > 1 ? cw.b : nullptr;
    RUN(c, mphip_conv3d_fwd_split(x.data.p, xr, wp, cw.b, o.t.data.p, n, cw.ci, cw.co, d, h, w, cw.k, prec, nullptr, 0, c.s));
    return o;
}

void ensure_stats(Ctx &c, ConvOut &y, int groups) {
    if (y.stats.off != (size_t)-1 && y.stats_groups == groups) return;
    const int n = y.t.n, ch = y.t.c, s = y.t.d * y.t.h * y.t.w;
    if (y.stats.off != (size_t)-1) give(c, y.stats);
    y.stats = take(c, (size_t)n * groups * 2 * sizeof(float));
    y.stats_groups = groups;
    if (y.splits > 1) {
        if ((size_t)(ch / groups) * s > STATS_SPLIT_MAX_SPAN) {
            if (c.rc == MPHIP_OK && !c.dry) {
                set_error("hot_slice: split-K GroupNorm span %zu floats > %zu (shape outside the planned schedule)", (size_t)(ch / groups) * s,
                          STATS_SPLIT_MAX_SPAN);
                c.rc = MPHIP_EINVAL;
            }
            return;
        }
        RUN(c, mphip_groupnorm_stats_split(y.t.data.p, y.splits, y.bias, y.stats.p, n, ch, s, groups, GN_EPS, c.s));
        return;
    }
    const size_t ws_bytes = mphip_groupnorm_workspace_bytes(n, ch, s, groups);
    Buf ws = take(c, ws_bytes);
    RUN(c, mphip_groupnorm_stats(y.t.data.p, y.stats.p, n, ch, s, groups, GN_EPS, ws.p, ws_bytes, c.s));
    give(c, ws);
}

T5 groupnorm_apply(Ctx &c, ConvOut &x, const Norm &nm, int groups, const ConvOut *res, bool relu, bool tanh_, bool pool2, int ud, int uh, int uw) {
    const int n = x.t.n, ch = x.t.c, d = x.t.d, h = x.t.h, w = x.t.w;
    const int rs = res ? res->splits : 1;
    const bool general = x.splits > 1 || rs > 1 || ud != 1 || uh != 1 || uw != 1;
    T5 y = pool2 ? new_t5(c, n, ch, d / 2, h / 2, w / 2, true) : new_t5(c, n, ch, d * ud, h * uh, w * uw, true);
    if (general)
        RUN(c, mphip_groupnorm_apply_split(x.t.data.p, x.splits, x.bias, x.stats.p, nm.gw, nm.gb, nm.w2, nm.b2, res ? res->t.data.p : nullptr, rs,
                                           res ? res->bias : nullptr, y.data.p, y.range.p, n, ch, d, h, w, groups, relu, tanh_, pool2, ud, uh, uw,
                                           c.s));
    else
        RUN(c, mphip_groupnorm_apply(x.t.data.p, x.stats.p, nm.gw, nm.gb, nm.w2, nm.b2, res ? res->t.data.p : nullptr, y.data.p, y.range.p, n, ch,
                                     d, h, w, groups, relu, tanh_, pool2, c.s));
    return y;
}

bool groupnorm_fused_ok(const ConvOut &x, int groups) {
    return (size_t)(x.t.c / groups) * x.t.d * x.t.h * x.t.w <= GN_FUSED_MAX_SPAN;
}

T5 groupnorm_small(Ctx &c, ConvOut &x, const Norm &nm, int groups, const ConvOut *res, bool relu, bool tanh_, int ud, int uh, int uw) {
    const int n = x.t.n, ch = x.t.c, d = x.t.d, h = x.t.h, w = x.t.w;
    T5 y = new_t5(c, n, ch, d * ud, h * uh, w * uw, false);
    RUN(c, mphip_groupnorm_small_fused(x.t.data.p, x.splits, x.bias, nm.gw, nm.gb, nm.w2, nm.b2, res ? res->t.data.p : nullptr, res ? res->splits : 1,
                                       res ? res->bias : nullptr, y.data.p, nullptr, n, ch, d, h, w, groups, GN_EPS, relu, tanh_, ud, uh, uw, c.s));
    return y;
}

bool gn_in_conv_ok(const Ctx &c, int n, int d, int h, int w, const ConvW &pc2) {
    if (c.p->precision != 1 || pc2.k != 3 || pc2.ci > 768) return false;
    return mphip_conv3d_supported(n, pc2.ci, pc2.co, d, h, w, pc2.k, 1) != 0;
}
bool gn_in_conv_ok(const Ctx &c, const ConvOut &y, const ConvW &pc2) { return gn_in_conv_ok(c, y.t.n, y.t.d, y.t.h, y.t.w, pc2); }

ConvOut conv3d_gn_in(Ctx &c, ConvOut &y, const Norm &nm, int groups, ConvW &pc2, int out_gn_groups) {
    const int n = y.t.n, ci = y.t.c, d = y.t.d, h = y.t.h, w = y.t.w;
    const bool have = y.table.off != (size_t)-1;
    Buf table = have ? y.table : take(c, (size_t)n * ci * 2 * sizeof(float));
    Buf xr = have ? y.table_range : take(c, MPHIP_RANGE_FLOATS * sizeof(float));
    y.table = Buf();
    y.table_range = Buf();
    if (!have) RUN(c, mphip_groupnorm_affine_table(y.stats.p, nm.gw, nm.gb, nm.w2, nm.b2, table.p, xr.p, n, ci, d * h * w, groups, c.s));
    const void *wp = packed(c, pc2, 1);
    const size_t ws_bytes = mphip_conv3d_gn_workspace_bytes(n, ci, pc2.co, d, h, w, pc2.k, 1, out_gn_groups);
    Buf ws = take(c, ws_bytes);
    ConvOut o;
    o.t = new_t5(c, n, pc2.co, d, h, w, false);
    o.stats = take(c, (size_t)n * out_gn_groups * 2 * sizeof(float));
// ... 94 lines not shown
    }
    for (int l = 0; l < L; ++l) res[l] = b[l]->identity ? as_convout(x[l]) : conv3d_split(*ln[l].c, x[l], b[l]->res, 0);
    if (tiny) {
        for (int l = 0; l < L; ++l) out[l] = groupnorm_small(*ln[l].c, y2[l], b[l]->n2, 32, &res[l], true, false, ud, uh, uw);
    } else {
        for (int l = 0; l < L; ++l) ensure_stats(*ln[l].c, y2[l], 32);
        for (int l = 0; l < L; ++l) out[l] = groupnorm_apply(*ln[l].c, y2[l], b[l]->n2, 32, &res[l], true, false, false, ud, uh, uw);
    }
    for (int l = 0; l < L; ++l) {
        give(*ln[l].c, y2[l]);
        if (!b[l]->identity) give(*ln[l].c, res[l]);
        give(*ln[l].c, x[l]);
        x[l] = out[l];
    }
}

template <int L>
void generator_coords(GenLane (&ln)[L], int B, Buf (&coords)[L]) {
    static const int UPS[4][3] = {{2, 2, 2}, {2, 2, 2}, {1, 2, 2}, {1, 2, 2}};
    Plan *p = ln[0].c->p;
    const int G = p->G;
    T5 x[L], em[L];
    ConvOut y[L];
    Buf theta[L];
    for (int l = 0; l < L; ++l) {
        Ctx &c = *ln[l].c;
        FlowFieldW &ff = ln[l].g->ff;
        if (!c.dry && !ff.kn_fresh) {
            hipLaunchKernelGGL(transpose_kernel, dim3(512 / 32, 2048 / 32), dim3(256), 0, c.s, ff.w1x1, ff.w1x1_kn, 2048, 512);
            if (c.rc == MPHIP_OK) c.rc = check_launch("hot_slice(transpose conv1x1)");
            RUN(c, mphip_small_gemm(ln[l].g->gamma, nullptr, ff.w1x1_kn, nullptr, ff.w_head, 512, 2048, 512, 512, 1, 2048, 1, c.s));
            ff.kn_fresh = true;
        }
        x[l] = new_t5(c, B, 512, 4, 1, 1, false);
        RUN(c, mphip_add_matmul(ln[l].z, ln[l].e, ff.w_head, ff.b1x1, x[l].data.p, B, 512, 2048, 0, c.s));
    }
    for (int i = 0; i < 4; ++i) resblock_ada<L>(ln, i, x, UPS[i][0], UPS[i][1], UPS[i][2]);
    static const bool ff_fused = !(getenv("MPHIP_FF_FUSED") && getenv("MPHIP_FF_FUSED")[0] == '0');
    const ConvW &co0 = ln[0].g->ff.conv_out;
    const bool out_fused = ff_fused && co0.ci == 32 && co0.co == 3 && co0.k == 3 && x[0].d == 16 && x[0].h == 16 && x[0].w == 16;
    if (out_fused) {
        for (int l = 0; l < L; ++l) {
            Ctx &c = *ln[l].c;
            FlowFieldW &ff = ln[l].g->ff;
            em[l] = new_t5(c, B, 3, 16, 16, 16, false);
            const size_t wsb = mphip_flowfield_out_workspace_bytes(B);
            Buf ws = take(c, wsb);
            RUN(c, mphip_flowfield_out(x[l].data.p, ff.conv_out.w, ff.conv_out.b, ff.gn.gw, ff.gn.gb, em[l].data.p, B, GN_EPS, ws.p, wsb, c.s));
            give(c, ws);
            give(c, x[l]);
        }
    } else {
    for (int l = 0; l < L; ++l) { y[l] = conv3d_split(*ln[l].c, x[l], ln[l].g->ff.conv_out, 0); give(*ln[l].c, x[l]); }
    if (groupnorm_fused_ok(y[0], 1)) {
        for (int l = 0; l < L; ++l) em[l] = groupnorm_small(*ln[l].c, y[l], ln[l].g->ff.gn, 1, nullptr, true, true, 1, 1, 1);
    } else {
        for (int l = 0; l < L; ++l) ensure_stats(*ln[l].c, y[l], 1);
        for (int l = 0; l < L; ++l) em[l] = groupnorm_apply(*ln[l].c, y[l], ln[l].g->ff.gn, 1, nullptr, true, true, false, 1, 1, 1);
    }
    for (int l = 0; l < L; ++l) give(*ln[l].c, y[l]);
    }
    for (int l = 0; l < L; ++l) {
        Ctx &c = *ln[l].c;
        theta[l] = take(c, (size_t)B * 12 * sizeof(float));
        RUN(c, mphip_rt_theta(ln[l].R, ln[l].t, theta[l].p, B, ln[l].g->invert, c.s));
    }
    for (int l = 0; l < L; ++l) {
        Ctx &c = *ln[l].c;
        coords[l] = take(c, (size_t)B * p->D * p->H * p->W * 3 * sizeof(float));
        if (p->H == G && p->W == G) {
            RUN(c, mphip_warp_field_coords(theta[l].p, em[l].data.p, p->aff_base, p->lin_d, p->lin_h, p->lin_w, coords[l].p, B, em[l].d, em[l].h, em[l].w,
                                           G, p->D, c.s));
        } else {
            T5 wf = new_t5(c, B, 3, G, G, G, false);
            RUN(c, mphip_warp_field_compose(theta[l].p, em[l].data.p, p->aff_base, wf.data.p, nullptr, nullptr, B, em[l].d, em[l].h, em[l].w, G, c.s));
            RUN(c, mphip_warp_coords(wf.data.p, p->lin_d, p->lin_h, p->lin_w, coords[l].p, B, p->D, p->H, p->W, G, G, G, c.s));
            give(c, wf);
        }
        give(c, theta[l]);
        give(c, em[l]);
    }
}

template <typename Hook>
T5 resblock(Ctx &c, ResBlock &b, T5 &x, bool pool_after, Hook hook) {
    ConvOut identity = b.identity ? as_convout(x) : conv3d_split(c, x, b.shortcut, 0);
    ConvOut y = conv3d_split(c, x, b.conv1, 32, &b.gn1, &b.conv2);
    hook();
    ensure_stats(c, y, 32);
    ConvOut y2;
    if (y.splits == 1 && gn_in_conv_ok(c, y, b.conv2)) {
        y2 = conv3d_gn_in(c, y, b.gn1, 32, b.conv2, 32);
        give(c, y);
    } else {
        T5 a = groupnorm_apply(c, y, b.gn1, 32, nullptr, true, false, false, 1, 1, 1);
        give(c, y);
        y2 = conv3d_split(c, a, b.conv2, 32);
        give(c, a);
    }
    ensure_stats(c, y2, 32);
    T5 out = groupnorm_apply(c, y2, b.gn2, 32, &identity, true, false, pool_after, 1, 1, 1);
    give(c, y2);
    if (!b.identity) give(c, identity);
    give(c, x);
    return out;
}

struct Roi {
    const int *box = nullptr;
    bool on = false;
    int tile[3] = {0, 0, 0};
};

T5 upsample2(Ctx &c, T5 &x, const Roi *roi = nullptr) {
    T5 y;
    y.n = x.n; y.c = x.c; y.d = 2 * x.d; y.h = 2 * x.h; y.w = 2 * x.w;
    y.data = take(c, y.numel() * sizeof(float));
    if (roi && roi->on)
        RUN(c, mphip_upsample_trilinear2_roi(x.data.p, y.data.p, roi->box, 0, x.n, x.c, x.d, x.h, x.w, roi->tile[0], roi->tile[1], roi->tile[2], c.s));
    else
        RUN(c, mphip_upsample_trilinear2(x.data.p, y.data.p, x.n * x.c, x.d, x.h, x.w, c.s));
    y.range = x.range;
    y.has_range = x.has_range;
    x.range = Buf();
    x.has_range = false;
    give(c, x.data);
    return y;
}

template <typename Hook, typename Tail>
T5 g3d(Ctx &c, T5 &x, bool external_out, float *out, Hook hook, Tail tail) {
    Plan *p = c.p;
    auto none = [] {};
    T5 t = resblock(c, p->down[0], x, true, hook);
    t = resblock(c, p->down[1], t, true, none);
    t = resblock(c, p->down[2], t, true, none);
    t = resblock(c, p->down[3], t, false, none);
    t = resblock(c, p->up[0], t, false, none);
    t = upsample2(c, t);
    t = resblock(c, p->up[1], t, false, none);
    t = upsample2(c, t);
    t = resblock(c, p->up[2], t, false, none);
    ConvW &cw = p->final_conv;
    Roi roi = tail();
    if (roi.on) roi.on = mphip_conv3d_roi_granule(t.n, cw.ci, cw.co, 2 * t.d, 2 * t.h, 2 * t.w, cw.k, precision_for(c, t.n, cw.ci, cw.co, 2 * t.d, 2 * t.h, 2 * t.w, cw.k), roi.tile) != 0;
    t = upsample2(c, t, &roi);
    const int prec = precision_for(c, t.n, cw.ci, cw.co, t.d, t.h, t.w, cw.k);
    const void *wp = packed(c, cw, prec);
    const float *xr = prec == 1 ? range_for(c, t) : nullptr;
    const size_t ws_bytes = roi.on ? mphip_conv3d_roi_workspace_bytes(t.n, cw.ci, cw.co, t.d, t.h, t.w, cw.k, prec)
                                   : mphip_conv3d_workspace_bytes(t.n, cw.ci, cw.co, t.d, t.h, t.w, cw.k, prec);
    Buf ws;
    if (ws_bytes) ws = take(c, ws_bytes);
    T5 y;
    y.n = t.n; y.c = cw.co; y.d = t.d; y.h = t.h; y.w = t.w;
    if (external_out) y.data.p = out; else y.data = take(c, y.numel() * sizeof(float));
    prof_arm(c, cw, t.d, t.h, t.w, roi.on ? 1 : 0);
    if (roi.on)
        RUN(c, mphip_conv3d_fwd_roi(t.data.p, xr, wp, cw.b, y.data.p, roi.box, 0, t.n, cw.ci, cw.co, t.d, t.h, t.w, cw.k, prec, ws.p, ws_bytes, c.s));
    else
        RUN(c, mphip_conv3d_fwd(t.data.p, xr, wp, cw.b, y.data.p, t.n, cw.ci, cw.co, t.d, t.h, t.w, cw.k, prec, ws.p, ws_bytes, c.s));
    give(c, ws);
    give(c, t);
    return y;
}

int run_slice(Plan *p, const void *vs, const float *es, const float *Rs, const float *ts, const float *zs, const float *Rd, const float *td,
              const float *zd, void *out, int B, void *workspace, size_t workspace_bytes, hipStream_t s, bool dry, size_t *need,
              int vs_dt = MPHIP_DTYPE_F32, int out_dt = MPHIP_DTYPE_F32) {
    const bool overlap = p->overlap && !dry;
    size_t side_bytes = 0, main_bytes = 0;
    if (!dry) {
        auto hit = p->slice_sizes.find(B);
        if (hit == p->slice_sizes.end()) {
            run_slice(p, nullptr, nullptr, nullptr, nullptr, nullptr, nullptr, nullptr, nullptr, nullptr, B, nullptr, 0, nullptr, true, nullptr);
            hit = p->slice_sizes.emplace(B, std::make_pair(p->main_arena.peak, p->side_arena.peak)).first;
        }
        main_bytes = hit->second.first;
        side_bytes = hit->second.second;
        if (workspace_bytes < main_bytes + side_bytes || !workspace) {
            set_error("hot_slice_forward: workspace %zu bytes < required %zu", workspace_bytes, main_bytes + side_bytes);
            return MPHIP_EWORKSPACE;
        }
    }
    p->main_arena.reset(workspace, dry ? 0 : main_bytes, dry);
    p->side_arena.reset(dry ? nullptr : (char *)workspace + main_bytes, dry ? 0 : side_bytes, dry);
// ... 437 lines not shown
```

megaportrait-hack_amd/model.py:

```python
from __future__ import annotations

import logging
import os
from typing import Optional

import torch
import torch.nn as nn
import torch.nn.functional as F

from . import autograd as ag
from . import ops

COMPRESS_DIM = 512
_C2D_EARLY = os.environ.get("MPHIP_C2D_EARLY", "0") == "1"


def _f32(*tensors):
    out = tuple(t.float() if isinstance(t, torch.Tensor) and t.is_floating_point() and t.dtype != torch.float32 else t
                for t in tensors)
    return out[0] if len(out) == 1 else out


def _autocast_policy(fn):
    import functools
# ... 310 lines not shown
        if train:
            x = ag.conv3d(x, self.conv3x3x3, _packs.get(self.conv3x3x3))
            x = ag.groupnorm(x, self.gn, relu=True, tanh=True)
            assert x.shape[1] == 3, f"Expected 3 channels after conv3x3x3, got {x.shape[1]}"
            return x
        if ops.flowfield_out_ok(tuple(x.shape), self.conv3x3x3) and self.gn.num_groups == 1:
            return ops.flowfield_out(x, self.conv3x3x3, self.gn)
        x = ops.conv3d_split(x, _packs.get(self.conv3x3x3))
        if ops.groupnorm_fused_ok(x, 1):
            x = ops.groupnorm_small(x, self.gn.weight, self.gn.bias, 1, self.gn.eps, relu=True, tanh=True)
        else:
            st = ops.groupnorm_stats(x, 1, self.gn.eps)
            x = ops.groupnorm_apply(x, st, self.gn.weight, self.gn.bias, 1, relu=True, tanh=True)
        assert x.shape[1] == 3, f"Expected 3 channels after conv3x3x3, got {x.shape[1]}"
        return x


class _WarpGenerator(_ModelDtype, nn.Module):
    _INVERT = False

    def __init__(self, num_channels):
        super().__init__()
        self.flowfield = FlowField()
        self.num_channels = COMPRESS_DIM
        self.adaptive_matrix_gamma = nn.Parameter(torch.randn(self.num_channels, self.num_channels))
        self.adaptive_matrix_beta = nn.Parameter(torch.randn(self.num_channels, self.num_channels))

    @_model_dtype_forward()
    def forward(self, R, t, z, e):
        assert R.shape == (z.shape[0], 3), f"Expected R shape (batch_size, 3), got {R.shape}"
        assert t.shape == (z.shape[0], 3), f"Expected t shape (batch_size, 3), got {t.shape}"
        assert z.shape == e.shape, f"Expected z and e to have the same shape, got {z.shape} and {e.shape}"
        R, t, z, e = _f32(R, t, z, e)
        if ag.needs_grad(self, R, t, z, e):
            s = ag.AddMatmulFn.apply(z, e, self.adaptive_matrix_gamma)
            em = self.flowfield(s.unsqueeze(-1).unsqueeze(-1), 0, 0)
            theta = ag.RtThetaFn.apply(R, t, self._INVERT)
            return ag.WarpFieldComposeFn.apply(theta, em, 64)
        em = self.flowfield.forward_from_codes(z, e, self.adaptive_matrix_gamma)
        theta = ops.rt_theta(R, t, self._INVERT)
        return ops.warp_field_compose(theta, em, 64)


class WarpGeneratorS2C(_WarpGenerator):
    _INVERT = True


class WarpGeneratorC2D(_WarpGenerator):
    _INVERT = False


class ResBlock3D(nn.Module):

    def __init__(self, in_channels, out_channels, upsample=False, scale_factors=(1, 1, 1)):
        super().__init__()
        self.upsample = upsample
        self.scale_factors = scale_factors
        self.conv1 = nn.Conv3d(in_channels, out_channels, kernel_size=3, padding=1)
        self.gn1 = nn.GroupNorm(num_groups=32, num_channels=out_channels)
        self.conv2 = nn.Conv3d(out_channels, out_channels, kernel_size=3, padding=1)
        self.gn2 = nn.GroupNorm(num_groups=32, num_channels=out_channels)
        self.shortcut = nn.Conv3d(in_channels, out_channels, kernel_size=1) if in_channels != out_channels else nn.Identity()

    def _forward_train(self, x):
        identity = x if isinstance(self.shortcut, nn.Identity) else ag.conv3d(x, self.shortcut, _packs.get(self.shortcut))
        y = ag.conv3d(x, self.conv1, _packs.get(self.conv1))
        y = ag.groupnorm(y, self.gn1, relu=True)
        y = ag.conv3d(y, self.conv2, _packs.get(self.conv2))
        return ag.groupnorm(y, self.gn2, residual=identity, relu=True)

    def forward(self, x, _pool_after: bool = False, _after_conv1=None):
        out = self._forward(x, _pool_after, _after_conv1)
        if self.upsample:
            out = _upsample_trilinear(out, self.scale_factors)
        return out

    def _forward(self, x, _pool_after: bool = False, _after_conv1=None):
        x = _f32(x)
        if ag.needs_grad(self, x):
            y = self._forward_train(x)
            if _after_conv1 is not None:
                _after_conv1()
            return ag.AvgPool2Fn.apply(y) if _pool_after else y
        identity = x if isinstance(self.shortcut, nn.Identity) else ops.conv3d_split(x, _packs.get(self.shortcut))
        y = ops.conv3d_split(x, _packs.get(self.conv1), gn_groups=32, gn_eps=self.gn1.eps)
        if _after_conv1 is not None:
            _after_conv1()
        st = ops.groupnorm_stats(y, 32, self.gn1.eps)
        pc2 = _packs.get(self.conv2)
        if y.splits == 1 and ops.gn_in_conv_ok(y.shape, pc2):
            y2, st2 = ops.conv3d_gn_in(y.data, st, self.gn1.weight, self.gn1.bias, 32, pc2, out_gn_groups=32,
                                       out_gn_eps=self.gn2.eps)
            y = ops.ConvOut(y2, 1, None, y.shape, st2, 32)
        else:
            a = ops.groupnorm_apply(y, st, self.gn1.weight, self.gn1.bias, 32, relu=True)
            y = ops.conv3d_split(a, pc2, gn_groups=32, gn_eps=self.gn2.eps)
        st = ops.groupnorm_stats(y, 32, self.gn2.eps)
        return ops.groupnorm_apply(y, st, self.gn2.weight, self.gn2.bias, 32, residual=identity, relu=True,
                                   pool2=_pool_after)


class G3d(_ModelDtype, nn.Module):

    def __init__(self, in_channels):
        super().__init__()
        self.downsampling = nn.Sequential(
            ResBlock3D(in_channels, 96), nn.AvgPool3d(kernel_size=2, stride=2),
            ResBlock3D(96, 192), nn.AvgPool3d(kernel_size=2, stride=2),
            ResBlock3D(192, 384), nn.AvgPool3d(kernel_size=2, stride=2),
            ResBlock3D(384, 768),
        )
        self.upsampling = nn.Sequential(
            ResBlock3D(768, 384), nn.Upsample(scale_factor=2, mode="trilinear", align_corners=True),
            ResBlock3D(384, 192), nn.Upsample(scale_factor=2, mode="trilinear", align_corners=True),
            ResBlock3D(192, 96), nn.Upsample(scale_factor=2, mode="trilinear", align_corners=True),
        )
        self.final_conv = nn.Conv3d(96, 96, kernel_size=3, padding=1)

    @_model_dtype_forward(cast_input=True)
    @_autocast_policy
    def forward(self, x, _after_first_conv=None, _final_roi=None):
        x = _f32(x)
        train = ag.needs_grad(self, x)
        up = ag.UpsampleTrilinear2Fn.apply if train else ops.upsample_trilinear2
        d = self.downsampling
        x = d[0](x, _pool_after=True, _after_conv1=_after_first_conv)
        x = d[2](x, _pool_after=True)
        x = d[4](x, _pool_after=True)
        x = d[6](x)
        u = self.upsampling
        x = up(u[0](x))
        x = up(u[2](x))
        x = up(u[4](x))
        if train:
            return ag.conv3d(x, self.final_conv, _packs.get(self.final_conv), roi=_final_roi)
        return ops.conv3d(x, _packs.get(self.final_conv))


class Eapp3DTail(_ModelDtype, nn.Module):

    _ORDER = ("resblock3D_96", "resblock3D_96_2", "resblock3D_96_1", "resblock3D_96_1_2", "resblock3D_96_2",
              "resblock3D_96_2_2")
    max_frames_per_pass = 64

    def __init__(self):
        super().__init__()
        self.resblock3D_96 = ResBlock3D_Adaptive(in_channels=96, out_channels=96)
        self.resblock3D_96_1 = ResBlock3D_Adaptive(in_channels=96, out_channels=96)
        self.resblock3D_96_1_2 = ResBlock3D_Adaptive(in_channels=96, out_channels=96)
        self.resblock3D_96_2 = ResBlock3D_Adaptive(in_channels=96, out_channels=96)
        self.resblock3D_96_2_2 = ResBlock3D_Adaptive(in_channels=96, out_channels=96)

    @_model_dtype_forward(cast_input=True, volume_input=True)
    @_autocast_policy
    def forward(self, out):
        out = _f32(out)
        vs = out.view(out.size(0), 96, 16, *out.shape[2:]) if out.dim() == 4 else out
        if vs.shape[0] > self.max_frames_per_pass and not ag.needs_grad(self, vs):
            step = int(self.max_frames_per_pass)
            return torch.cat([self.forward(vs[i:i + step]) for i in range(0, vs.shape[0], step)], dim=0)
        for name in self._ORDER:
            vs = getattr(self, name)(vs)
        return vs


def eapp_tail(owner: nn.Module, vs):
    blocks = {name: getattr(owner, name) for name in Eapp3DTail._ORDER}
    dts = {p.dtype for b in blocks.values() for p in b.parameters()}
    if dts == {torch.float32}:
        owner.__dict__.pop("_mphip_tail_twin", None)
        for name in Eapp3DTail._ORDER:
            vs = blocks[name](vs)
        return vs
    if len(dts) > 1:
        raise RuntimeError(f"{type(owner).__name__}: the 3-D tail's parameters mix dtypes ({', '.join(sorted(str(d) for d in dts))}); convert "
                           "the module as a whole with .float(), .half() or .bfloat16()")
    dt = dts.pop()
    _refuse_half_training(nn.ModuleList(blocks.values()), dt, vs)

    def build():
# ... 1057 lines not shown
```

megaportrait-hack_amd/ops.py:

```python
from __future__ import annotations

import ctypes
from typing import Optional, Tuple, Union

import os as _os

import torch

from . import _lib

_P = ctypes.c_void_p


def _ptr(t: Optional[torch.Tensor]):
    return None if t is None else _P(t.data_ptr())


def _stream():
    return _P(torch.cuda.current_stream().cuda_stream)


def _req(t: torch.Tensor, name: str, dtype=torch.float32) -> torch.Tensor:
    if not isinstance(t, torch.Tensor) or not t.is_cuda:
        raise RuntimeError(f"{name}: expected a CUDA tensor (the HIP path has no CPU fallback), got "
# ... 514 lines not shown
    y = torch.empty((n, pc.co, d, h, w), dtype=torch.float32, device=x.device)

    def launch():
        if gn_groups:
            _lib.check(lib.mphip_conv3d_gn_fwd(_ptr(x), _ptr(xr), _ptr(wp), _ptr(pc.bias), _ptr(y), _ptr(stats), n, ci, pc.co, d, h, w,
                                               pc.k, prec, gn_groups, gn_eps, _ptr(ws), ws_bytes, _stream()),
                       "mphip_conv3d_gn_fwd")
        else:
            _lib.check(lib.mphip_conv3d_fwd(_ptr(x), _ptr(xr), _ptr(wp), _ptr(pc.bias), _ptr(y), n, ci, pc.co, d, h, w, pc.k, prec,
                                            _ptr(ws), ws_bytes, _stream()), "mphip_conv3d_fwd")
        return y

    y = _conv_hook(x, pc, launch) if _conv_hook is not None else launch()
    return (y, stats) if gn_groups else y


_GNIN_ENABLED = _os.environ.get("MPHIP_GN_IN_CONV", "1") != "0"


def gn_in_conv_ok(x_shape, pc: "PackedConv") -> bool:
    if not _GNIN_ENABLED or _default_precision != 1 or pc.k != 3 or pc.ci > 768:
        return False
    n, ci, d, h, w = x_shape
    return bool(_lib.load().mphip_conv3d_supported(n, ci, pc.co, d, h, w, pc.k, 1))


def conv3d_gn_in(x: torch.Tensor, stats: torch.Tensor, gamma, beta, groups: int, pc: "PackedConv", w2=None, b2=None,
                 relu: bool = True, out_gn_groups: Optional[int] = None, out_gn_eps: float = 1e-5):
    x = _req(x, "x")
    n, ci, d, h, w = x.shape
    lib = _lib.load()
    gamma, beta = _req(gamma.detach(), "gamma"), _req(beta.detach(), "beta")
    if w2 is not None:
        w2, b2 = _req(w2.detach(), "w2").reshape(-1), _req(b2.detach(), "b2").reshape(-1)
    table = torch.empty((n, ci, 2), dtype=torch.float32, device=x.device)
    xr = new_range(x.device)
    _lib.check(lib.mphip_groupnorm_affine_table(_ptr(stats), _ptr(gamma), _ptr(beta), _ptr(w2), _ptr(b2), _ptr(table), _ptr(xr), n,
                                                ci, d * h * w, groups, _stream()), "mphip_groupnorm_affine_table")
    wp = pc.packed(1)
    if out_gn_groups:
        ws_bytes = lib.mphip_conv3d_gn_workspace_bytes(n, ci, pc.co, d, h, w, pc.k, 1, out_gn_groups)
        out_stats = torch.empty((n * out_gn_groups, 2), dtype=torch.float32, device=x.device)
    else:
        ws_bytes = lib.mphip_conv3d_workspace_bytes(n, ci, pc.co, d, h, w, pc.k, 1)
        out_stats = None
    ws = torch.empty((ws_bytes + 7) // 8, dtype=torch.float64, device=x.device) if ws_bytes else None
    y = torch.empty((n, pc.co, d, h, w), dtype=torch.float32, device=x.device)

    def launch():
        if out_gn_groups:
            _lib.check(lib.mphip_conv3d_gnin_gn_fwd(_ptr(x), _ptr(table), _ptr(xr), int(relu), _ptr(wp), _ptr(pc.bias), _ptr(y), _ptr(out_stats),
                                                    n, ci, pc.co, d, h, w, pc.k, 1, out_gn_groups, out_gn_eps, _ptr(ws), ws_bytes,
                                                    _stream()), "mphip_conv3d_gnin_gn_fwd")
        else:
            _lib.check(lib.mphip_conv3d_gnin_fwd(_ptr(x), _ptr(table), _ptr(xr), int(relu), _ptr(wp), _ptr(pc.bias), _ptr(y), n, ci, pc.co, d,
                                                 h, w, pc.k, 1, _ptr(ws), ws_bytes, _stream()), "mphip_conv3d_gnin_fwd")
        return y

    y = _conv_hook(x, pc, launch) if _conv_hook is not None else launch()
    return (y, out_stats) if out_gn_groups else y


class ConvOut:

    __slots__ = ("data", "splits", "bias", "shape", "stats", "stats_groups")

    def __init__(self, data, splits, bias, shape, stats=None, stats_groups=0):
        self.data, self.splits, self.bias, self.shape = data, splits, bias, shape
        self.stats, self.stats_groups = stats, stats_groups


def conv3d_split(x: torch.Tensor, pc: PackedConv, precision: Optional[int] = None, gn_groups: Optional[int] = None,
                 gn_eps: float = 1e-5) -> ConvOut:
    x = _req(x, "x")
    if x.dim() != 5 or x.shape[1] != pc.ci:
        raise RuntimeError(f"conv3d: input {tuple(x.shape)} does not match Ci={pc.ci}")
    n, ci, d, h, w = x.shape
    lib = _lib.load()
    prec = _default_precision if precision is None else precision
    if prec != 0 and not lib.mphip_conv3d_supported(n, ci, pc.co, d, h, w, pc.k, prec):
        prec = 0
    splits = lib.mphip_conv3d_splits(n, ci, pc.co, d, h, w, pc.k, prec)
    shape = (n, pc.co, d, h, w)
    elems = n * pc.co * d * h * w
    if splits > 1 and (elems > _SPLIT_CHAIN_MAX_ELEMS or (splits >= _SPLIT_CHAIN_MAX_SPLITS and splits * elems > _SPLIT_CHAIN_MAX_SLAB_ELEMS)):
        if gn_groups:
            y, st = conv3d(x, pc, precision=prec, gn_groups=gn_groups, gn_eps=gn_eps)
            return ConvOut(y, 1, None, shape, st, gn_groups)
        return ConvOut(conv3d(x, pc, precision=prec), 1, None, shape)
    if gn_groups and splits == 1 and prec == 1:
        y, st = conv3d(x, pc, precision=prec, gn_groups=gn_groups, gn_eps=gn_eps)
        return ConvOut(y, 1, None, shape, st, gn_groups)
    out = torch.empty((splits,) + shape if splits > 1 else shape, dtype=torch.float32, device=x.device)
    wp = pc.packed(prec)
    xr = _range_for(x) if prec == 1 else None

    def launch():
        _lib.check(lib.mphip_conv3d_fwd_split(_ptr(x), _ptr(xr), _ptr(wp), _ptr(pc.bias), _ptr(out), n, ci, pc.co, d, h, w, pc.k,
                                              prec, None, 0, _stream()), "mphip_conv3d_fwd_split")
        return out

    if _conv_hook is not None:
        _conv_hook(x, pc, launch)
    else:
        launch()
    return ConvOut(out, splits, pc.bias if splits > 1 else None, shape)


_SPLIT_CHAIN_MAX_ELEMS = 1 << 18
_SPLIT_CHAIN_MAX_SPLITS = 16
_SPLIT_CHAIN_MAX_SLAB_ELEMS = 1 << 20
_STATS_SPLIT_MAX_SPAN = 65536


def _finish(co: ConvOut) -> torch.Tensor:
    if co.splits == 1:
        return co.data
    y = co.data.sum(dim=0)
    return y if co.bias is None else y + co.bias.view(1, -1, 1, 1, 1)


def groupnorm_stats(x, groups: int, eps: float = 1e-5) -> torch.Tensor:
    lib = _lib.load()
    if isinstance(x, ConvOut) and x.stats is not None and x.stats_groups == groups:
        return x.stats
    if isinstance(x, ConvOut):
        n, c, d, h, w = x.shape
        s = d * h * w
        if x.splits > 1 and (c // groups) * s <= _STATS_SPLIT_MAX_SPAN:
            stats = torch.empty((n * groups, 2), dtype=torch.float32, device=x.data.device)
            _lib.check(lib.mphip_groupnorm_stats_split(_ptr(x.data), x.splits, _ptr(x.bias), _ptr(stats), n, c, s, groups, eps,
                                                       _stream()), "mphip_groupnorm_stats_split")
            return stats
        x = _finish(x)
    x = _req(x, "x")
    n, c = x.shape[0], x.shape[1]
    s = x.numel() // (n * c)
    stats = torch.empty((n * groups, 2), dtype=torch.float32, device=x.device)
    ws_bytes = lib.mphip_groupnorm_workspace_bytes(n, c, s, groups)
    if ws_bytes == 0:
        raise RuntimeError(f"groupnorm_stats: bad dims C={c} G={groups}")
    ws = torch.empty(ws_bytes // 8, dtype=torch.float64, device=x.device)
    _lib.check(lib.mphip_groupnorm_stats(_ptr(x), _ptr(stats), n, c, s, groups, eps, _ptr(ws), ws_bytes, _stream()),
               "mphip_groupnorm_stats")
    return stats


def groupnorm_apply(x, stats, gamma, beta, groups: int, w2=None, b2=None, residual=None, relu=False, tanh=False,
                    pool2=False, up=(1, 1, 1)) -> torch.Tensor:
    lib = _lib.load()
    xs = x.splits if isinstance(x, ConvOut) else 1
    rs = residual.splits if isinstance(residual, ConvOut) else 1
    xt = x.data if isinstance(x, ConvOut) else x
    rt = residual.data if isinstance(residual, ConvOut) else residual
    shape = x.shape if isinstance(x, ConvOut) else tuple(x.shape)
    if len(shape) != 5:
        raise RuntimeError("groupnorm_apply: expected a 5-D NCDHW tensor")
    n, c, d, h, w = shape
    xt = _req(xt, "x")
    gamma, beta = _req(gamma.detach(), "gamma"), _req(beta.detach(), "beta")
    if w2 is not None:
        w2, b2 = _req(w2.detach(), "w2").reshape(-1), _req(b2.detach(), "b2").reshape(-1)
    if rt is not None:
        rt = _req(rt, "residual")
        rshape = residual.shape if isinstance(residual, ConvOut) else tuple(residual.shape)
        if tuple(rshape) != tuple(shape):
            raise RuntimeError("groupnorm_apply: residual shape mismatch")
    up = tuple(int(u) for u in up)
    general = xs > 1 or rs > 1 or up != (1, 1, 1)
    if pool2:
        oshape = (n, c, d // 2, h // 2, w // 2)
    else:
        oshape = (n, c, d * up[0], h * up[1], w * up[2])
    y = torch.empty(oshape, dtype=torch.float32, device=xt.device)
    rng = new_range(xt.device) if _RANGES_ENABLED else None
    if general:
        xb = x.bias if isinstance(x, ConvOut) else None
        rb = residual.bias if isinstance(residual, ConvOut) else None
        _lib.check(lib.mphip_groupnorm_apply_split(_ptr(xt), xs, _ptr(xb), _ptr(stats), _ptr(gamma), _ptr(beta), _ptr(w2), _ptr(b2),
                                                   _ptr(rt), rs, _ptr(rb), _ptr(y), _ptr(rng), n, c, d, h, w, groups, int(relu),
                                                   int(tanh), int(pool2), up[0], up[1], up[2], _stream()),
                   "mphip_groupnorm_apply_split")
    else:
        _lib.check(lib.mphip_groupnorm_apply(_ptr(xt), _ptr(stats), _ptr(gamma), _ptr(beta), _ptr(w2), _ptr(b2), _ptr(rt),
                                             _ptr(y), _ptr(rng), n, c, d, h, w, groups, int(relu), int(tanh), int(pool2),
                                             _stream()), "mphip_groupnorm_apply")
    return tag_range(y, rng)


_GN_FUSED_MAX_SPAN = 12288


_GN_SMALL_ENABLED = _os.environ.get("MPHIP_GN_SMALL", "1") != "0"


def groupnorm_fused_ok(x, groups: int) -> bool:
    if not _GN_SMALL_ENABLED:
        return False
    shape = x.shape if isinstance(x, ConvOut) else tuple(x.shape)
    n, c, d, h, w = shape
    return (c // groups) * d * h * w <= _GN_FUSED_MAX_SPAN


def groupnorm_small(x, gamma, beta, groups: int, eps: float = 1e-5, w2=None, b2=None, residual=None, relu=False,
                    tanh=False, up=(1, 1, 1)) -> torch.Tensor:
    lib = _lib.load()
    xs = x.splits if isinstance(x, ConvOut) else 1
    rs = residual.splits if isinstance(residual, ConvOut) else 1
    xt = _req(x.data if isinstance(x, ConvOut) else x, "x")
    rt = residual.data if isinstance(residual, ConvOut) else residual
    shape = x.shape if isinstance(x, ConvOut) else tuple(x.shape)
    n, c, d, h, w = shape
    gamma, beta = _req(gamma.detach(), "gamma"), _req(beta.detach(), "beta")
    if w2 is not None:
        w2, b2 = _req(w2.detach(), "w2").reshape(-1), _req(b2.detach(), "b2").reshape(-1)
    if rt is not None:
        rt = _req(rt, "residual")
    xb = x.bias if isinstance(x, ConvOut) else None
    rb = residual.bias if isinstance(residual, ConvOut) else None
    up = tuple(int(u) for u in up)
    y = torch.empty((n, c, d * up[0], h * up[1], w * up[2]), dtype=torch.float32, device=xt.device)
    _lib.check(lib.mphip_groupnorm_small_fused(_ptr(xt), xs, _ptr(xb), _ptr(gamma), _ptr(beta), _ptr(w2), _ptr(b2), _ptr(rt), rs,
                                               _ptr(rb), _ptr(y), None, n, c, d, h, w, groups, eps, int(relu), int(tanh), up[0],
                                               up[1], up[2], _stream()), "mphip_groupnorm_small_fused")
    return y


_FF_FUSED = _os.environ.get("MPHIP_FF_FUSED", "1") != "0"


def flowfield_conv_gn_ok(x_shape, conv, res_conv=None, groups: int = 32) -> bool:
    if not _FF_FUSED or len(x_shape) != 5:
        return False
    n, ci, d, h, w = x_shape
    cr = res_conv.weight.shape[1] if res_conv is not None else 0
    return bool(_lib.load().mphip_flowfield_conv_gn_supported(ci, conv.weight.shape[0], d, h, w, cr, groups))


def flowfield_conv_gn(x, conv, norm, res_x=None, res_conv=None, relu=True, up=(1, 1, 1)) -> torch.Tensor:
    x = _req(x, "x")
    n, ci, d, h, w = x.shape
    co = conv.weight.shape[0]
    wt, bs = _req(conv.weight.detach(), "conv.weight"), (_req(conv.bias.detach(), "conv.bias") if conv.bias is not None else None)
    g, b = _req(norm.group_norm.weight.detach(), "gamma"), _req(norm.group_norm.bias.detach(), "beta")
    w2, b2 = _req(norm.weight.detach(), "w2").reshape(-1), _req(norm.bias.detach(), "b2").reshape(-1)
    rx = rw = rb = None
    cr = 0
    if res_conv is not None:
        rx = _req(res_x, "res_x")
        rw = _req(res_conv.weight.detach(), "res_conv.weight")
        rb = _req(res_conv.bias.detach(), "res_conv.bias") if res_conv.bias is not None else None
        cr = rw.shape[1]
    up = tuple(int(u) for u in up)
    y = torch.empty((n, co, d * up[0], h * up[1], w * up[2]), dtype=torch.float32, device=x.device)
    _lib.check(_lib.load().mphip_flowfield_conv_gn(_ptr(x), _ptr(wt), _ptr(bs), _ptr(g), _ptr(b), _ptr(w2), _ptr(b2), _ptr(rx), _ptr(rw),
                                                   _ptr(rb), _ptr(y), n, ci, co, d, h, w, cr, up[0], up[1], up[2], norm.num_groups,
                                                   norm.group_norm.eps, int(relu), _stream()), "mphip_flowfield_conv_gn")
    return y


def flowfield_out_ok(x_shape, conv) -> bool:
    return _FF_FUSED and tuple(x_shape[1:]) == (32, 16, 16, 16) and tuple(conv.weight.shape) == (3, 32, 3, 3, 3)


def flowfield_out(x, conv, gn) -> torch.Tensor:
    x = _req(x, "x")
    n = x.shape[0]
    lib = _lib.load()
    wt, bs = _req(conv.weight.detach(), "conv.weight"), (_req(conv.bias.detach(), "conv.bias") if conv.bias is not None else None)
    g, b = _req(gn.weight.detach(), "gamma"), _req(gn.bias.detach(), "beta")
    ws_bytes = lib.mphip_flowfield_out_workspace_bytes(n)
    ws = torch.empty((ws_bytes + 7) // 8, dtype=torch.float64, device=x.device)
# ... 612 lines not shown
```

Baseline: 3262.

## Fuse resblock 1x1 shortcut conv into GroupNorm+residual+ReLU(+pool) epilogue

Adds a fused kernel mode where the 1x1 f16x3 shortcut convolution computes its output and, in its epilogue, reads conv2's output and GN stats, applies GroupNorm, adds the shortcut result as the residual, applies ReLU, and optionally 2x2x2 average-pools. This removes the separate shortcut output tensor write/read and the standalone groupnorm_apply launch in non-identity resblocks. It adds an extra strided read of y2 inside the conv kernel, a brick-shaped column mapping when pooling, and register pressure in the epilogue.

```diff
diff --git a/include/mphip.h b/include/mphip.h
--- a/include/mphip.h
+++ b/include/mphip.h
@@ -70,6 +70,10 @@
                               const float *gamma, const float *beta, const float *w2, const float *b2, float *table, float *table_range,
                               int N, int Ci, int Co, int D, int H, int W, int k, int precision, int gn_groups, float gn_eps,
                               void *workspace, size_t workspace_bytes, void *stream);
+int mphip_conv3d_k1_gn_res_supported(int N, int Ci, int Co, int D, int H, int W, int groups, int pool2);
+int mphip_conv3d_k1_gn_res_fwd(const float *x, const float *x_range, const void *w_packed, const float *bias, const float *y2,
+                               const float *stats, const float *gamma, const float *beta, float *out, float *out_range, int N, int Ci,
+                               int Co, int D, int H, int W, int groups, int relu, int pool2, void *stream);
 int mphip_flowfield_conv_gn_supported(int Ci, int Co, int D, int H, int W, int Cr, int groups);
 int mphip_flowfield_conv_gn(const float *x, const float *w, const float *b, const float *gamma, const float *beta, const float *w2,
                             const float *b2, const float *res_x, const float *res_w, const float *res_b, float *y, int N, int Ci, int Co,
diff --git a/megaportrait-hack_amd/_lib.py b/megaportrait-hack_amd/_lib.py
--- a/megaportrait-hack_amd/_lib.py
+++ b/megaportrait-hack_amd/_lib.py
@@ -48,6 +48,8 @@
     "mphip_conv3d_fwd": (_i, [_p, _p, _p, _p, _p, _i, _i, _i, _i, _i, _i, _i, _i, _p, _sz, _p]),
     "mphip_conv3d_gn_workspace_bytes": (_sz, [_i, _i, _i, _i, _i, _i, _i, _i, _i]),
     "mphip_conv3d_gn_fwd": (_i, [_p, _p, _p, _p, _p, _p, _i, _i, _i, _i, _i, _i, _i, _i, _i, ctypes.c_float, _p, _sz, _p]),
+    "mphip_conv3d_k1_gn_res_supported": (_i, [_i] * 8),
+    "mphip_conv3d_k1_gn_res_fwd": (_i, [_p] * 10 + [_i] * 9 + [_p]),
     "mphip_conv3d_gn_table_fwd": (_i, [_p] * 12 + [_i] * 9 + [ctypes.c_float, _p, _sz, _p]),
     "mphip_conv3d_time_next_launch": (None, [_p, _p]),
     "mphip_groupnorm_affine_table": (_i, [_p, _p, _p, _p, _p, _p, _p, _i, _i, _i, _i, _p]),
diff --git a/megaportrait-hack_amd/csrc/conv3d.hip b/megaportrait-hack_amd/csrc/conv3d.hip
--- a/megaportrait-hack_amd/csrc/conv3d.hip
+++ b/megaportrait-hack_amd/csrc/conv3d.hip
@@ -6,6 +6,7 @@
 
 #include "mphip_common.h"
 #include "mphip_conv.h"
+#include "mphip_gn.h"
 
 namespace mphip {
 
@@ -865,6 +866,26 @@
                       workspace_bytes, stream, nullptr, 0, 0, &t);
 }
 
+extern "C" int mphip_conv3d_k1_gn_res_supported(int N, int Ci, int Co, int D, int H, int W, int groups, int pool2) {
+    if (N <= 0 || Ci <= 0 || Co <= 0 || D <= 0 || H <= 0 || W <= 0) return 0;
+    return f16x3_k1_finish_supported(f16x3_switches(), N, Ci, Co, D, H, W, groups, pool2) ? 1 : 0;
+}
+
+extern "C" int mphip_conv3d_k1_gn_res_fwd(const float *x, const float *x_range, const void *w_packed, const float *bias, const float *y2,
+                                          const float *stats, const float *gamma, const float *beta, float *out, float *out_range, int N,
+                                          int Ci, int Co, int D, int H, int W, int groups, int relu, int pool2, void *stream) {
+    MPHIP_REQUIRE(x && x_range && w_packed && y2 && stats && gamma && beta && out, "conv3d_k1_gn_res_fwd: null pointer");
+    MPHIP_REQUIRE(N > 0 && Ci > 0 && Co > 0 && D > 0 && H > 0 && W > 0, "conv3d_k1_gn_res_fwd: bad dims");
+    MPHIP_REQUIRE(groups > 0 && Co % groups == 0, "conv3d_k1_gn_res_fwd: Co=%d not divisible into %d groups", Co, groups);
+    const F16x3Switches sw = f16x3_switches();
+    MPHIP_REQUIRE(f16x3_k1_finish_supported(sw, N, Ci, Co, D, H, W, groups, pool2),
+                  "conv3d_k1_gn_res_fwd: shape not fused (query mphip_conv3d_k1_gn_res_supported; run mphip_conv3d_fwd + mphip_groupnorm_apply)");
+    GnParams fin{};
+    fin.x = y2; fin.stats = stats; fin.gamma = gamma; fin.beta = beta; fin.y = out; fin.range = out_range;
+    fin.C = Co; fin.cpg = Co / groups; fin.relu = relu;
+    return f16x3_launch_k1_finish(sw, x, w_packed, bias, N, Ci, Co, D, H, W, x_range, fin, pool2, (hipStream_t)stream);
+}
+
 extern "C" int mphip_conv3d_gnin_fwd(const float *x, const float *in_affine, const float *x_range, int in_relu, const void *w_packed,
                                      const float *bias, float *y, int N, int Ci, int Co, int D, int H, int W, int k,
                                      int precision, void *workspace, size_t workspace_bytes, void *stream) {
diff --git a/megaportrait-hack_amd/csrc/conv3d_f16x3.hip b/megaportrait-hack_amd/csrc/conv3d_f16x3.hip
--- a/megaportrait-hack_amd/csrc/conv3d_f16x3.hip
+++ b/megaportrait-hack_amd/csrc/conv3d_f16x3.hip
@@ -7,6 +7,7 @@
 #include "mphip_common.h"
 #include "mphip_conv.h"
 #include "mphip_f16x3.h"
+#include "mphip_gn.h"
 
 namespace mphip {
 
@@ -659,26 +660,99 @@
     f16x3_pack_k1_body(w, out, hdr_in, hdr_out, Co, Ci, transposed, blockIdx.x, gridDim.x);
 }
 
-template <int KS, int NTT = 2>
+struct K1Channel {
+    float mean, rstd, g, b;
+};
+template <int FIN, int NT>
+__device__ __forceinline__ unsigned k1_finish(const GnParams &fin, const float (&yv)[NT], const float (&res)[NT], const K1Channel &ch, bool live,
+                                              size_t plane, int DHW, int rl, int tfloats, bool owner, int pool_off) {
+    float v[NT];
+#pragma unroll
+    for (int t = 0; t < NT; ++t) v[t] = gn_value(fin, yv[t], ch.mean, ch.rstd, ch.g, ch.b, 1.0f, 0.0f, false, res[t], true);
+    unsigned mbits = 0;
+    if (FIN == 2) {
+        float s = 0.0f;
+#pragma unroll
+        for (int t = 0; t < NT; ++t) {
+            const float w1 = __shfl_xor(v[t], 1, 64), h1 = __shfl_xor(v[t], 16, 64), h1w1 = __shfl_xor(v[t], 17, 64);
+            s += v[t];
+            s += w1;
+            s += h1;
+            s += h1w1;
+        }
+        if (owner) {
+            if (live) fin.y[plane * (DHW / 8) + pool_off] = s / 8.0f;
+            mbits = range_bits(s / 8.0f);
+        }
+    } else {
+#pragma unroll
+        for (int t = 0; t < NT; ++t) {
+            if (live) fin.y[plane * DHW + rl + t * tfloats] = v[t];
+            mbits = max(mbits, range_bits(v[t]));
+        }
+    }
+    return mbits;
+}
+
+template <int KS, int NTT = 2, int FIN = 0>
 __global__ void __launch_bounds__(KS == 1 ? 256 : 64 * KS) __attribute__((amdgpu_waves_per_eu(2)))
 conv3d_k1_f16x3_kernel(const float *__restrict__ x, const _Float16 *__restrict__ wslabs, const float *__restrict__ whdr,
                        const float *__restrict__ bias, float *__restrict__ y, int N, int Ci, int Co, int DHW, unsigned x_bytes,
-                       const float *__restrict__ x_range) {
+                       const float *__restrict__ x_range, GnParams fin, int H, int W) {
     constexpr int MT = 3, NT = NTT;
+    fin.tanh_ = 0;
+    static_assert(FIN != 2 || NTT == 2, "the pooled epilogue pairs the two column tiles of a wave");
     float x_scale = X_SCALE, x_unscale = 1.0f / X_SCALE;
     if (x_range) range_scale_block(x_range, x_scale, x_unscale);
     const int lane = threadIdx.x & 63, wave = threadIdx.x >> 6;
     const int j = lane & 31, kg = lane >> 5;
-    const long v0 = (KS == 1 ? (long)blockIdx.x * 4 + wave : (long)blockIdx.x) * (NT * 32);
-    if (v0 >= (long)N * DHW) return;
+    long v0 = (KS == 1 ? (long)blockIdx.x * 4 + wave : (long)blockIdx.x) * (NT * 32);
+    bool live = true;
+    if (v0 >= (long)N * DHW) {
+        if (FIN == 0) return;
+        live = false;
+        v0 = 0;
+    }
     const int n = (int)(v0 / DHW), r0 = (int)(v0 - (long)n * DHW);
+    int rl = r0 + j, tfloats = 32, pool_off = 0;
+    if (FIN == 2) {
+        const int bw = W / 16, bh = H / 2, brick = r0 / 64;
+        const int wq = brick % bw, hq = (brick / bw) % bh, dq = brick / (bw * bh);
+        rl = ((2 * dq) * H + 2 * hq + (j >> 4)) * W + wq * 16 + (j & 15);
+        tfloats = H * W;
+        pool_off = (dq * bh + hq) * (W / 2) + wq * 8 + ((j & 15) >> 1);
+    }
+    const bool owner = (j & 17) == 0;
     const int cot = blockIdx.y, nchunks = Ci / F16X3_KC;
     const int cps = (nchunks + KS - 1) / KS;
     const int c_begin = KS == 1 ? 0 : wave * cps, c_end = KS == 1 ? nchunks : min(nchunks, c_begin + cps);
     __amdgpu_buffer_rsrc_t rsrc = __builtin_amdgcn_make_buffer_rsrc((void *)x, 0, (int)x_bytes, 0x00020000);
-    const unsigned vbase = (unsigned)((((long)n * Ci + kg * 8) * DHW + r0 + j) * 4);
-    const unsigned cstride = (unsigned)DHW * 4u;
+    const unsigned vbase = (unsigned)((((long)n * Ci + kg * 8) * DHW + rl) * 4);
+    const unsigned cstride = (unsigned)DHW * 4u, tstride = (unsigned)tfloats * 4u;
     const _Float16 *wl = wslabs + (size_t)cot * nchunks * K1_SLAB_HALFS + (kg * F16X3_COT + j) * 8;
+    const int co0 = cot * F16X3_COT;
+    constexpr int FIN_TILES = KS == 1 ? 4 : 1;
+    __shared__ float fin_prm[FIN ? (FIN_TILES * 2 + 3) * F16X3_COT : 1];
+    if (FIN) {
+        if (KS == 1 || wave == 0) {
+            float *mr = fin_prm + (KS == 1 ? wave : 0) * 2 * F16X3_COT;
+            for (int c = lane; c < F16X3_COT; c += 64) {
+                const int grp = n * (fin.C / fin.cpg) + (co0 + c) / fin.cpg;
+                mr[2 * c] = fin.stats[grp * 2];
+                mr[2 * c + 1] = fin.stats[grp * 2 + 1];
+            }
+        }
+        float *gb = fin_prm + FIN_TILES * 2 * F16X3_COT;
+        for (int c = threadIdx.x; c < F16X3_COT; c += blockDim.x) {
+            gb[c] = fin.gamma[co0 + c];
+            gb[F16X3_COT + c] = fin.beta[co0 + c];
+            gb[2 * F16X3_COT + c] = bias ? bias[co0 + c] : 0.0f;
+        }
+        __syncthreads();
+    }
+    const float *fin_mr = fin_prm + (KS == 1 ? wave : 0) * 2 * F16X3_COT, *fin_gb = fin_prm + FIN_TILES * 2 * F16X3_COT;
+    const size_t plane0 = (size_t)n * Co + co0;
+#define K1_CHANNEL(c_) K1Channel{fin_mr[2 * (c_)], fin_mr[2 * (c_) + 1], fin_gb[c_], fin_gb[F16X3_COT + (c_)]}
 
     f32x16 acc[MT][NT];
 #pragma unroll
@@ -696,7 +770,7 @@
         const unsigned soff_ = (unsigned)((long)(c_) * F16X3_KC * DHW * 4);                                           \
         _Pragma("unroll") for (int t = 0; t < NT; ++t)                                                                \
             _Pragma("unroll") for (int e = 0; e < 8; ++e)                                                             \
-                xv[set][t][e] = buf_load_f(rsrc, vbase + (unsigned)t * 128u + (unsigned)e * cstride, soff_);          \
+                xv[set][t][e] = buf_load_f(rsrc, vbase + (unsigned)t * tstride + (unsigned)e * cstride, soff_);              \
         const _Float16 *ws_ = wl + (size_t)(c_) * K1_SLAB_HALFS;                                                      \
         _Pragma("unroll") for (int m = 0; m < MT; ++m) {                                                              \
             ah[set][m] = *reinterpret_cast<const half8 *>(ws_ + m * 32 * 8);                                          \
@@ -737,8 +811,29 @@
 #undef K1_LOAD
 #undef K1_MFMA
     const float unscale = whdr[0] * x_unscale;
-    const int co0 = cot * F16X3_COT;
-    if (KS == 1) {
+    unsigned mbits = 0;
+    if (KS == 1 && FIN) {
+        float yv[2][16][NT];
+#define K1_Y2(m_)                                                                                                      \
+    _Pragma("unroll") for (int reg = 0; reg < 16; ++reg)                                                               \
+        _Pragma("unroll") for (int t = 0; t < NT; ++t)                                                                 \
+            yv[(m_) & 1][reg][t] = fin.x[(plane0 + (m_) * 32 + (reg & 3) + 8 * (reg >> 2) + 4 * kg) * DHW + rl + t * tfloats];
+        K1_Y2(0)
+#pragma unroll
+        for (int m = 0; m < MT; ++m) {
+            if (m + 1 < MT) K1_Y2(m + 1)
+#pragma unroll
+            for (int reg = 0; reg < 16; ++reg) {
+                const int c = m * 32 + (reg & 3) + 8 * (reg >> 2) + 4 * kg;
+                const float bv = fin_gb[2 * F16X3_COT + c];
+                float res[NT];
+#pragma unroll
+                for (int t = 0; t < NT; ++t) res[t] = acc[m][t][reg] * unscale + bv;
+                mbits = max(mbits, k1_finish<FIN, NT>(fin, yv[m & 1][reg], res, K1_CHANNEL(c), live, plane0 + c, DHW, rl, tfloats, owner, pool_off));
+            }
+        }
+#undef K1_Y2
+    } else if (KS == 1) {
 #pragma unroll
         for (int m = 0; m < MT; ++m) {
 #pragma unroll
@@ -754,29 +849,60 @@
         __shared__ float red[KS > 1 ? KS : 1][NT * 16 * 64];
 #pragma unroll
         for (int m = 0; m < MT; ++m) {
+            constexpr int NQ = 16 / KS;
+            float yq[NQ][NT];
+            if (FIN) {
+#pragma unroll
+                for (int i = 0; i < NQ; ++i) {
+                    const int reg = wave + i * KS;
+#pragma unroll
+                    for (int t = 0; t < NT; ++t) yq[i][t] = fin.x[(plane0 + m * 32 + (reg & 3) + 8 * (reg >> 2) + 4 * kg) * DHW + rl + t * tfloats];
+                }
+            }
 #pragma unroll
             for (int t = 0; t < NT; ++t)
 #pragma unroll
                 for (int reg = 0; reg < 16; ++reg) red[wave][(t * 16 + reg) * 64 + lane] = acc[m][t][reg];
             __syncthreads();
-            for (int q = wave; q < NT * 16; q += KS) {
-                const int t = q >> 4, reg = q & 15;
-                float sum = red[0][q * 64 + lane];
-#pragma unroll
-                for (int k = 1; k < KS; ++k) sum += red[k][q * 64 + lane];
-                const int co = co0 + m * 32 + (reg & 3) + 8 * (reg >> 2) + 4 * kg;
-                const float bv = bias ? bias[co] : 0.0f;
-                y[((size_t)n * Co + co) * DHW + r0 + j + t * 32] = sum * unscale + bv;
+            if (FIN) {
+#pragma unroll
+                for (int i = 0; i < NQ; ++i) {
+                    const int reg = wave + i * KS;
+                    const int c = m * 32 + (reg & 3) + 8 * (reg >> 2) + 4 * kg;
+                    const float bv = fin_gb[2 * F16X3_COT + c];
+                    float res[NT];
+#pragma unroll
+                    for (int t = 0; t < NT; ++t) {
+                        float sum = red[0][(t * 16 + reg) * 64 + lane];
+#pragma unroll
+                        for (int k = 1; k < KS; ++k) sum += red[k][(t * 16 + reg) * 64 + lane];
+                        res[t] = sum * unscale + bv;
+                    }
+                    mbits = max(mbits, k1_finish<FIN, NT>(fin, yq[i], res, K1_CHANNEL(c), live, plane0 + c, DHW, rl, tfloats, owner, pool_off));
+                }
+            } else {
+                for (int q = wave; q < NT * 16; q += KS) {
+                    const int t = q >> 4, reg = q & 15;
+                    float sum = red[0][q * 64 + lane];
+#pragma unroll
+                    for (int k = 1; k < KS; ++k) sum += red[k][q * 64 + lane];
+                    const int co = co0 + m * 32 + (reg & 3) + 8 * (reg >> 2) + 4 * kg;
+                    const float bv = bias ? bias[co] : 0.0f;
+                    y[((size_t)n * Co + co) * DHW + r0 + j + t * 32] = sum * unscale + bv;
+                }
             }
             __syncthreads();
         }
     }
+    if (FIN && !live) sat_ = 0;
     if (__builtin_amdgcn_ballot_w64(sat_ != 0) != 0) {
         unsigned tot = sat_;
 #pragma unroll
         for (int sft = 32; sft >= 1; sft >>= 1) tot += __shfl_xor(tot, sft, 64);
         if (lane == 0) atomicAdd(&g_f16x3_saturated, (unsigned long long)tot);
     }
+#undef K1_CHANNEL
+    if (FIN && fin.range) range_note_block(mbits, fin.range, blockIdx.y * gridDim.x + blockIdx.x, gridDim.x * gridDim.y);
 }
 
 static int f16x3_k1_ksplit(const F16x3Switches &sw, int N, int Ci, int Co, int DHW) {
@@ -865,27 +991,63 @@
     return check_launch("pack_conv_weights(f16x3)");
 }
 
-int f16x3_launch_k1(const F16x3Switches &sw, const float *x, const void *wpacked, const float *bias, float *dst, int N, int Ci, int Co,
-                    int DHW, const float *x_range, hipStream_t s) {
+struct K1Geometry {
+    int ks;
+    bool nt1;
+    dim3 grid;
+    unsigned block;
+};
+static K1Geometry f16x3_k1_geometry(const F16x3Switches &sw, int N, int Ci, int Co, int DHW) {
+    K1Geometry g;
+    const long waves = (long)N * DHW / 64;
+    g.ks = f16x3_k1_ksplit(sw, N, Ci, Co, DHW);
+    g.nt1 = g.ks == 1 && (sw.k1_nt >= 0 ? sw.k1_nt == 1 : waves * (Co / F16X3_COT) <= 1024);
+    g.grid = dim3((unsigned)(g.ks > 1 ? waves : g.nt1 ? (2 * waves + 3) / 4 : (waves + 3) / 4), Co / F16X3_COT);
+    g.block = g.ks > 1 ? 64u * g.ks : 256u;
+    return g;
+}
+
+template <int FIN>
+static void f16x3_launch_k1_mode(const K1Geometry &g, const float *x, const void *wpacked, const float *bias, float *dst, int N, int Ci, int Co,
+                                 int DHW, const float *x_range, const GnParams &fin, int H, int W, hipStream_t s) {
     const float *hdr = (const float *)wpacked;
     const _Float16 *slabs = (const _Float16 *)((const char *)wpacked + 16);
     const unsigned xb = (unsigned)((size_t)N * Ci * DHW * 4);
-    const long waves = (long)N * DHW / 64;
-    const int ks = f16x3_k1_ksplit(sw, N, Ci, Co, DHW);
-    const bool nt1 = ks == 1 && (sw.k1_nt >= 0 ? sw.k1_nt == 1 : waves * (Co / F16X3_COT) <= 1024);
-    if (ks == 8)
-        hipLaunchKernelGGL(conv3d_k1_f16x3_kernel<8>, dim3((unsigned)waves, Co / F16X3_COT), dim3(512), 0, s, x, slabs, hdr, bias, dst, N, Ci,
-                           Co, DHW, xb, x_range);
-    else if (ks == 4)
-        hipLaunchKernelGGL(conv3d_k1_f16x3_kernel<4>, dim3((unsigned)waves, Co / F16X3_COT), dim3(256), 0, s, x, slabs, hdr, bias, dst, N, Ci,
-                           Co, DHW, xb, x_range);
-    else if (nt1)
-        hipLaunchKernelGGL((conv3d_k1_f16x3_kernel<1, 1>), dim3((unsigned)((2 * waves + 3) / 4), Co / F16X3_COT), dim3(256), 0, s, x, slabs, hdr,
-                           bias, dst, N, Ci, Co, DHW, xb, x_range);
-    else
-        hipLaunchKernelGGL(conv3d_k1_f16x3_kernel<1>, dim3((unsigned)((waves + 3) / 4), Co / F16X3_COT), dim3(256), 0, s, x, slabs, hdr, bias,
-                           dst, N, Ci, Co, DHW, xb, x_range);
+    if (g.ks == 8)
+        hipLaunchKernelGGL((conv3d_k1_f16x3_kernel<8, 2, FIN>), g.grid, dim3(g.block), 0, s, x, slabs, hdr, bias, dst, N, Ci, Co, DHW, xb, x_range,
+                           fin, H, W);
+    else if (g.ks == 4)
+        hipLaunchKernelGGL((conv3d_k1_f16x3_kernel<4, 2, FIN>), g.grid, dim3(g.block), 0, s, x, slabs, hdr, bias, dst, N, Ci, Co, DHW, xb, x_range,
+                           fin, H, W);
+    else if (g.nt1) {
+        if constexpr (FIN != 2)
+            hipLaunchKernelGGL((conv3d_k1_f16x3_kernel<1, 1, FIN>), g.grid, dim3(g.block), 0, s, x, slabs, hdr, bias, dst, N, Ci, Co, DHW, xb,
+                               x_range, fin, H, W);
+    } else
+        hipLaunchKernelGGL((conv3d_k1_f16x3_kernel<1, 2, FIN>), g.grid, dim3(g.block), 0, s, x, slabs, hdr, bias, dst, N, Ci, Co, DHW, xb, x_range,
+                           fin, H, W);
+}
+
+int f16x3_launch_k1(const F16x3Switches &sw, const float *x, const void *wpacked, const float *bias, float *dst, int N, int Ci, int Co,
+                    int DHW, const float *x_range, hipStream_t s) {
+    f16x3_launch_k1_mode<0>(f16x3_k1_geometry(sw, N, Ci, Co, DHW), x, wpacked, bias, dst, N, Ci, Co, DHW, x_range, GnParams{}, 0, 0, s);
     return check_launch("conv3d_fwd(f16x3, k=1)");
+}
+
+bool f16x3_k1_finish_supported(const F16x3Switches &sw, int N, int Ci, int Co, int D, int H, int W, int groups, int pool2) {
+    if (sw.finish_off || !f16x3_supported(sw, N, Ci, Co, D, H, W, 1) || groups <= 0 || Co % groups != 0) return false;
+    const K1Geometry g = f16x3_k1_geometry(sw, N, Ci, Co, D * H * W);
+    if ((size_t)g.grid.x * g.grid.y > RANGE_MAX_PARTS) return false;
+    if (pool2 && (g.nt1 || D % 2 != 0 || H % 2 != 0 || W % 16 != 0)) return false;
+    return true;
+}
+
+int f16x3_launch_k1_finish(const F16x3Switches &sw, const float *x, const void *wpacked, const float *bias, int N, int Ci, int Co, int D, int H,
+                           int W, const float *x_range, const GnParams &fin, int pool2, hipStream_t s) {
+    const K1Geometry g = f16x3_k1_geometry(sw, N, Ci, Co, D * H * W);
+    if (pool2) f16x3_launch_k1_mode<2>(g, x, wpacked, bias, nullptr, N, Ci, Co, D * H * W, x_range, fin, H, W, s);
+    else f16x3_launch_k1_mode<1>(g, x, wpacked, bias, nullptr, N, Ci, Co, D * H * W, x_range, fin, H, W, s);
+    return check_launch("conv3d_k1_gn_res_fwd(f16x3)");
 }
 
 int f16x3_launch(const F16x3Switches &sw, const F16x3Plan &p, const float *x, const void *wpacked, const float *bias, float *dst, int N, int Ci,
diff --git a/megaportrait-hack_amd/csrc/conv3d_f16x3_plan.hip b/megaportrait-hack_amd/csrc/conv3d_f16x3_plan.hip
--- a/megaportrait-hack_amd/csrc/conv3d_f16x3_plan.hip
+++ b/megaportrait-hack_amd/csrc/conv3d_f16x3_plan.hip
@@ -30,6 +30,7 @@
     sw.wino_pp = !pp ? 1 : pp[0] == '0' ? 0 : pp[0] == '2' ? 2 : 1;
     sw.k1_ks = (int)num("MPHIP_F16X3_K1_KS", 0);
     sw.k1_min_voxels = num("MPHIP_F16X3_K1_MIN", 1024);
+    sw.finish_off = zero("MPHIP_SHORTCUT_FINISH");
     return sw;
 }
 
diff --git a/megaportrait-hack_amd/csrc/mphip_conv.h b/megaportrait-hack_amd/csrc/mphip_conv.h
--- a/megaportrait-hack_amd/csrc/mphip_conv.h
+++ b/megaportrait-hack_amd/csrc/mphip_conv.h
@@ -42,6 +42,7 @@
     int wino_pp;
     int k1_ks;
     long k1_min_voxels;
+    bool finish_off;
     bool old_splits;
     bool xcd_on;
     bool wino_nopack;
@@ -81,6 +82,10 @@
 size_t f16x3_packed_bytes_k1(int Co, int Ci);
 int f16x3_launch_k1(const F16x3Switches &sw, const float *x, const void *wpacked, const float *bias, float *dst, int N, int Ci, int Co,
                     int DHW, const float *x_range, hipStream_t s);
+struct GnParams;
+bool f16x3_k1_finish_supported(const F16x3Switches &sw, int N, int Ci, int Co, int D, int H, int W, int groups, int pool2);
+int f16x3_launch_k1_finish(const F16x3Switches &sw, const float *x, const void *wpacked, const float *bias, int N, int Ci, int Co, int D, int H,
+                           int W, const float *x_range, const GnParams &fin, int pool2, hipStream_t s);
 int f16x3_pack(const float *w_oidhw, void *out, int Co, int Ci, int k, int transposed, const void *header_from, hipStream_t s);
 struct PackJob {
     const float *w;
diff --git a/megaportrait-hack_amd/csrc/mphip_gn.h b/megaportrait-hack_amd/csrc/mphip_gn.h
--- /dev/null
+++ b/megaportrait-hack_amd/csrc/mphip_gn.h
@@ -0,0 +1,24 @@
+#pragma once
+#include "mphip_common.h"
+
+namespace mphip {
+
+struct GnParams {
+    const float *x, *stats, *gamma, *beta, *w2, *b2, *residual;
+    float *y;
+    int C, cpg;
+    int relu, tanh_;
+    float *range;
+};
+
+__device__ __forceinline__ float gn_value(const GnParams &p, float xv, float mean, float rstd, float g, float b,
+                                          float w2, float b2, bool has2, float res, bool has_res) {
+    float v = (xv - mean) * rstd * g + b;
+    if (has2) v = v * w2 + b2;
+    if (has_res) v += res;
+    if (p.relu) v = fmaxf(v, 0.0f);
+    if (p.tanh_) v = tanhf(v);
+    return v;
+}
+
+}
diff --git a/megaportrait-hack_amd/csrc/norm.hip b/megaportrait-hack_amd/csrc/norm.hip
--- a/megaportrait-hack_amd/csrc/norm.hip
+++ b/megaportrait-hack_amd/csrc/norm.hip
@@ -2,6 +2,7 @@
 
 #include "mphip_common.h"
 #include "mphip_conv.h"
+#include "mphip_gn.h"
 #include "mphip_resample.h"
 
 namespace mphip {
@@ -195,24 +196,6 @@
         }
     }
     if (tbl.table && tbl.range) range_note_block(mbits, tbl.range, blockIdx.x, gridDim.x);
-}
-
-struct GnParams {
-    const float *x, *stats, *gamma, *beta, *w2, *b2, *residual;
-    float *y;
-    int C, cpg;
-    int relu, tanh_;
-    float *range;
-};
-
-__device__ __forceinline__ float gn_value(const GnParams &p, float xv, float mean, float rstd, float g, float b,
-                                          float w2, float b2, bool has2, float res, bool has_res) {
-    float v = (xv - mean) * rstd * g + b;
-    if (has2) v = v * w2 + b2;
-    if (has_res) v += res;
-    if (p.relu) v = fmaxf(v, 0.0f);
-    if (p.tanh_) v = tanhf(v);
-    return v;
 }
 
 template <int VW>
diff --git a/megaportrait-hack_amd/csrc/plan.hip b/megaportrait-hack_amd/csrc/plan.hip
--- a/megaportrait-hack_amd/csrc/plan.hip
+++ b/megaportrait-hack_amd/csrc/plan.hip
@@ -263,13 +263,20 @@
     return o;
 }
 
+int conv3d_split_slabs(const Ctx &c, int n, const ConvW &cw, int d, int h, int w) {
+    const int splits = mphip_conv3d_splits(n, cw.ci, cw.co, d, h, w, cw.k, precision_for(c, n, cw.ci, cw.co, d, h, w, cw.k));
+    const size_t elems = (size_t)n * cw.co * d * h * w;
+    if (splits > 1 && (elems > SPLIT_CHAIN_MAX_ELEMS || (splits >= SPLIT_CHAIN_MAX_SPLITS && (size_t)splits * elems > SPLIT_CHAIN_MAX_SLAB_ELEMS)))
+        return 1;
+    return splits;
+}
+
 ConvOut conv3d_split(Ctx &c, T5 &x, ConvW &cw, int gn_groups, const Norm *nm = nullptr, const ConvW *next = nullptr) {
     const int n = x.n, d = x.d, h = x.h, w = x.w;
     const int prec = precision_for(c, n, cw.ci, cw.co, d, h, w, cw.k);
     const int splits = mphip_conv3d_splits(n, cw.ci, cw.co, d, h, w, cw.k, prec);
     const size_t elems = (size_t)n * cw.co * d * h * w;
-    if (splits > 1 && (elems > SPLIT_CHAIN_MAX_ELEMS || (splits >= SPLIT_CHAIN_MAX_SPLITS && (size_t)splits * elems > SPLIT_CHAIN_MAX_SLAB_ELEMS)))
-        return conv3d(c, x, cw, gn_groups, nm, next);
+    if (splits > 1 && conv3d_split_slabs(c, n, cw, d, h, w) == 1) return conv3d(c, x, cw, gn_groups, nm, next);
     if (gn_groups && splits == 1 && prec == 1) return conv3d(c, x, cw, gn_groups, nm, next);
     const void *wp = packed(c, cw, prec);
     const float *xr = prec == 1 ? range_for(c, x) : nullptr;
@@ -530,9 +537,26 @@
     }
 }
 
+bool shortcut_finish_ok(const Ctx &c, const ResBlock &b, const T5 &x, bool pool_after) {
+    if (b.identity || c.p->precision != 1 || !mphip_conv3d_k1_gn_res_supported(x.n, b.shortcut.ci, b.shortcut.co, x.d, x.h, x.w, 32, pool_after)) return false;
+    const bool gn_in = conv3d_split_slabs(c, x.n, b.conv1, x.d, x.h, x.w) == 1 && gn_in_conv_ok(c, x.n, x.d, x.h, x.w, b.conv2);
+    return gn_in || conv3d_split_slabs(c, x.n, b.conv2, x.d, x.h, x.w) == 1;
+}
+
+T5 conv3d_k1_gn_res(Ctx &c, T5 &x, ConvW &cw, ConvOut &y2, const Norm &nm, int groups, bool relu, bool pool2) {
+    const int n = x.n, d = x.d, h = x.h, w = x.w;
+    const void *wp = packed(c, cw, 1);
+    const float *xr = range_for(c, x);
+    T5 out = pool2 ? new_t5(c, n, cw.co, d / 2, h / 2, w / 2, true) : new_t5(c, n, cw.co, d, h, w, true);
+    RUN(c, mphip_conv3d_k1_gn_res_fwd(x.data.p, xr, wp, cw.b, y2.t.data.p, y2.stats.p, nm.gw, nm.gb, out.data.p, out.range.p, n, cw.ci, cw.co, d, h, w,
+                                      groups, relu, pool2, c.s));
+    return out;
+}
+
 template <typename Hook>
 T5 resblock(Ctx &c, ResBlock &b, T5 &x, bool pool_after, Hook hook) {
-    ConvOut identity = b.identity ? as_convout(x) : conv3d_split(c, x, b.shortcut, 0);
+    const bool finish = shortcut_finish_ok(c, b, x, pool_after);
+    ConvOut identity = b.identity ? as_convout(x) : finish ? ConvOut() : conv3d_split(c, x, b.shortcut, 0);
     ConvOut y = conv3d_split(c, x, b.conv1, 32, &b.gn1, &b.conv2);
     hook();
     ensure_stats(c, y, 32);
@@ -547,9 +571,10 @@
         give(c, a);
     }
     ensure_stats(c, y2, 32);
-    T5 out = groupnorm_apply(c, y2, b.gn2, 32, &identity, true, false, pool_after, 1, 1, 1);
+    T5 out = finish ? conv3d_k1_gn_res(c, x, b.shortcut, y2, b.gn2, 32, true, pool_after)
+                    : groupnorm_apply(c, y2, b.gn2, 32, &identity, true, false, pool_after, 1, 1, 1);
     give(c, y2);
-    if (!b.identity) give(c, identity);
+    if (!b.identity && !finish) give(c, identity);
     give(c, x);
     return out;
 }
diff --git a/megaportrait-hack_amd/model.py b/megaportrait-hack_amd/model.py
--- a/megaportrait-hack_amd/model.py
+++ b/megaportrait-hack_amd/model.py
@@ -416,12 +416,14 @@
             if _after_conv1 is not None:
                 _after_conv1()
             return ag.AvgPool2Fn.apply(y) if _pool_after else y
-        identity = x if isinstance(self.shortcut, nn.Identity) else ops.conv3d_split(x, _packs.get(self.shortcut))
+        pc2 = _packs.get(self.conv2)
+        psc = None if isinstance(self.shortcut, nn.Identity) else _packs.get(self.shortcut)
+        finish = psc is not None and ops.shortcut_finish_ok(x.shape, psc, _packs.get(self.conv1), pc2, _pool_after)
+        identity = x if psc is None else None if finish else ops.conv3d_split(x, psc)
         y = ops.conv3d_split(x, _packs.get(self.conv1), gn_groups=32, gn_eps=self.gn1.eps)
         if _after_conv1 is not None:
             _after_conv1()
         st = ops.groupnorm_stats(y, 32, self.gn1.eps)
-        pc2 = _packs.get(self.conv2)
         if y.splits == 1 and ops.gn_in_conv_ok(y.shape, pc2):
             y2, st2 = ops.conv3d_gn_in(y.data, st, self.gn1.weight, self.gn1.bias, 32, pc2, out_gn_groups=32,
                                        out_gn_eps=self.gn2.eps)
@@ -430,6 +432,8 @@
             a = ops.groupnorm_apply(y, st, self.gn1.weight, self.gn1.bias, 32, relu=True)
             y = ops.conv3d_split(a, pc2, gn_groups=32, gn_eps=self.gn2.eps)
         st = ops.groupnorm_stats(y, 32, self.gn2.eps)
+        if finish:
+            return ops.conv3d_k1_gn_res(x, psc, y.data, st, self.gn2.weight, self.gn2.bias, 32, relu=True, pool2=_pool_after)
         return ops.groupnorm_apply(y, st, self.gn2.weight, self.gn2.bias, 32, residual=identity, relu=True,
                                    pool2=_pool_after)
 
diff --git a/megaportrait-hack_amd/ops.py b/megaportrait-hack_amd/ops.py
--- a/megaportrait-hack_amd/ops.py
+++ b/megaportrait-hack_amd/ops.py
@@ -620,8 +620,7 @@
         prec = 0
     splits = lib.mphip_conv3d_splits(n, ci, pc.co, d, h, w, pc.k, prec)
     shape = (n, pc.co, d, h, w)
-    elems = n * pc.co * d * h * w
-    if splits > 1 and (elems > _SPLIT_CHAIN_MAX_ELEMS or (splits >= _SPLIT_CHAIN_MAX_SPLITS and splits * elems > _SPLIT_CHAIN_MAX_SLAB_ELEMS)):
+    if splits > 1 and conv3d_split_slabs(x.shape, pc, prec) == 1:
         if gn_groups:
             y, st = conv3d(x, pc, precision=prec, gn_groups=gn_groups, gn_eps=gn_eps)
             return ConvOut(y, 1, None, shape, st, gn_groups)
@@ -643,6 +642,19 @@
     else:
         launch()
     return ConvOut(out, splits, pc.bias if splits > 1 else None, shape)
+
+
+def conv3d_split_slabs(x_shape, pc: PackedConv, precision: Optional[int] = None) -> int:
+    n, ci, d, h, w = x_shape
+    lib = _lib.load()
+    prec = _default_precision if precision is None else precision
+    if prec != 0 and not lib.mphip_conv3d_supported(n, ci, pc.co, d, h, w, pc.k, prec):
+        prec = 0
+    splits = lib.mphip_conv3d_splits(n, ci, pc.co, d, h, w, pc.k, prec)
+    elems = n * pc.co * d * h * w
+    if splits > 1 and (elems > _SPLIT_CHAIN_MAX_ELEMS or (splits >= _SPLIT_CHAIN_MAX_SPLITS and splits * elems > _SPLIT_CHAIN_MAX_SLAB_ELEMS)):
+        return 1
+    return splits
 
 
 _SPLIT_CHAIN_MAX_ELEMS = 1 << 18
@@ -726,6 +738,43 @@
     return tag_range(y, rng)
 
 
+def conv3d_k1_gn_res_ok(x_shape, pc: PackedConv, groups: int, pool2: bool = False) -> bool:
+    if _default_precision != 1 or pc.k != 1:
+        return False
+    n, ci, d, h, w = x_shape
+    return bool(_lib.load().mphip_conv3d_k1_gn_res_supported(n, ci, pc.co, d, h, w, groups, int(pool2)))
+
+
+def shortcut_finish_ok(x_shape, shortcut: PackedConv, conv1: PackedConv, conv2: PackedConv, pool2: bool) -> bool:
+    if not conv3d_k1_gn_res_ok(x_shape, shortcut, 32, pool2):
+        return False
+    mid = (x_shape[0], conv1.co) + tuple(x_shape[2:])
+    return (conv3d_split_slabs(x_shape, conv1) == 1 and gn_in_conv_ok(mid, conv2)) or conv3d_split_slabs(mid, conv2) == 1
+
+
+def conv3d_k1_gn_res(x: torch.Tensor, pc: PackedConv, y2: torch.Tensor, stats: torch.Tensor, gamma, beta, groups: int, relu: bool = True,
+                     pool2: bool = False) -> torch.Tensor:
+    x, y2 = _req(x, "x"), _req(y2, "y2")
+    n, ci, d, h, w = x.shape
+    if ci != pc.ci or tuple(y2.shape) != (n, pc.co, d, h, w):
+        raise RuntimeError(f"conv3d_k1_gn_res: x {tuple(x.shape)} / y2 {tuple(y2.shape)} do not match the conv {pc.ci} -> {pc.co}")
+    lib = _lib.load()
+    gamma, beta = _req(gamma.detach(), "gamma"), _req(beta.detach(), "beta")
+    wp = pc.packed(1)
+    xr = _range_for(x)
+    out = torch.empty((n, pc.co, d // 2, h // 2, w // 2) if pool2 else (n, pc.co, d, h, w), dtype=torch.float32, device=x.device)
+    rng = new_range(x.device) if _RANGES_ENABLED else None
+
+    def launch():
+        _lib.check(lib.mphip_conv3d_k1_gn_res_fwd(_ptr(x), _ptr(xr), _ptr(wp), _ptr(pc.bias), _ptr(y2), _ptr(stats), _ptr(gamma), _ptr(beta),
+                                                  _ptr(out), _ptr(rng), n, ci, pc.co, d, h, w, groups, int(relu), int(pool2), _stream()),
+                   "mphip_conv3d_k1_gn_res_fwd")
+        return out
+
+    out = _conv_hook(x, pc, launch) if _conv_hook is not None else launch()
+    return tag_range(out, rng)
+
+
 _GN_FUSED_MAX_SPAN = 12288
 
 
```

Measured after the change: 3307 (median of 6 runs). 1.01x the previous value.
